# huggingface/open-muse

Measured on AMD Instinct MI355X. Metric: images/sec/node (MaskGit train step, 256^2, bs=64/GPU), higher is better.
Workload: dtype bf16 (transformer GEMM/attention operands; f32 accumulate, residual, norms, loss) + bf16x3 tokenizer (f32 activations, f32-class products as 3 bf16 MFMAs); parity of this mode was not measured in this run (a --full run measures it); 1 GPU; MaskGit train step: MaskGitVQGAN f16-256 encode (bf16x3) + cosine mask + MaskGitTransformer config B (configs/imagenet.yaml: hidden 768, 24 layers, 16 heads, vocab 2048, seq 257) fwd+bwd (bf16 MFMA, f32 accum/residual) + AdamW; global_batch=64, per_gpu_batch=64, resolution=256, seq_len=257, parallelism=dp1, vqgan_dtype=bf16x3, random_init=True, wgrad_stream=True

## Files before the change

### include/muse_hip.h

```cpp
#ifndef MUSE_HIP_H
#define MUSE_HIP_H
#include <stdint.h>

#ifdef __cplusplus
extern "C" {
#endif

enum { MUSE_F32 = 0, MUSE_BF16 = 1, MUSE_F16 = 2  };
enum { MUSE_ERR_BAD_ARG = -1, MUSE_ERR_ALIGN = -2, MUSE_ERR_UNSUPPORTED = -3 };

int muse_version(void);

typedef struct muse_gemm_desc {
  const void* A;
  const void* B;
  void* C;
  const void* bias;
  const void* rowvec;
  const void* residual;
  int32_t dtype;
  int32_t out_dtype;
  int32_t layout_a, layout_b;
  int32_t M, N, K;
  int32_t batch, zdiv;
// ... 32 lines not shown
int muse_colsum(const float* in, float* out, int32_t rows, int32_t cols, int32_t accumulate, void* stream);
int muse_add_rowvec(float* x, const float* b, int64_t rows, int32_t cols, void* stream);
int muse_bias_grad_rows_per_block(void);
int muse_bias_grad_partial(const void* dy, int32_t dtype, float* partial, int64_t rows, int32_t cols, int64_t ld, void* stream);

int muse_softmax_fwd(const void* x, void* y, int32_t dtype, int64_t rows, int32_t cols, int64_t ld, void* stream);
int muse_softmax_bwd(const void* p, const void* dp, void* ds, int32_t dtype, int64_t rows, int32_t cols, int64_t ld,
                     void* stream);

typedef struct muse_attn_desc {
  const void* q;
  const void* k;
  const void* v;
  void* o;
  int64_t ldq, ldk, ldv, ldo;
  int64_t bsq, bsk, bsv, bso;
  int32_t batch, heads, head_dim, seq_q, seq_kv;
  float alpha;
} muse_attn_desc;
int muse_attention_seq_pad(int32_t seq);
int muse_attention_fwd_ex(const muse_attn_desc* d, float* lse, void* stream);
int muse_attention_bwd_ex(const muse_attn_desc* d, const void* d_o, int64_t lddo, int64_t bsdo, const float* lse, float* dsum,
                          void* dq, int64_t lddq, int64_t bsdq, void* dk, int64_t lddk, int64_t bsdk, void* dv, int64_t lddv,
                          int64_t bsdv, void* stream);
int muse_attention_x3_fwd(const muse_attn_desc* d, float* lse, void* o_planes, int64_t o_lo, int32_t half, float scale, int32_t* stats,
                          void* stream);
int muse_attention_x3_bwd(const muse_attn_desc* d, const void* d_o, int64_t lddo, int64_t bsdo, const float* lse, void* dq,
                          int64_t lddq, int64_t bsdq, void* dk, int64_t lddk, int64_t bsdk, void* dv, int64_t lddv, int64_t bsdv,
                          void* dq_planes, int64_t dq_lo, void* dk_planes, int64_t dk_lo, void* dv_planes, int64_t dv_lo, int32_t half,
                          float scale, int32_t* stats, void* stream);
int muse_attention_x3_fwd_stream(const muse_attn_desc* d, float* lse, void* o_planes, int64_t o_lo, int32_t half, float scale,
                                 int32_t* stats, void* stream);
int muse_attention_x3_bwd_stream(const muse_attn_desc* d, const float* d_o, int64_t lddo, int64_t bsdo, const float* lse, float* dsum,
                                 float* dq, int64_t lddq, int64_t bsdq, float* dk, int64_t lddk, int64_t bsdk, float* dv, int64_t lddv,
                                 int64_t bsdv, void* dq_planes, int64_t dq_lo, void* dk_planes, int64_t dk_lo, void* dv_planes, int64_t dv_lo,
                                 int32_t half, float scale, int32_t* stats, void* stream);
int muse_attention_x3_merge(const float* part, int64_t part_stride, const float* lp, int64_t lp_stride, int32_t nk, float* out, float* lse,
                            void* out_planes, int64_t out_lo, int32_t batch, int32_t seq, int32_t heads, int32_t half, float scale,
                            int32_t* stats, void* stream);
int muse_sum_parts_strided(const float* parts, int64_t part_stride, int32_t n, int64_t rows, int32_t cols, float* out, int64_t ldo,
                           int32_t accumulate, void* stream);
int muse_attention_fwd(const void* qkv, void* ctx, float* lse, int32_t batch, int32_t seq, int32_t heads,
                       int32_t head_dim, float alpha, void* stream);
int muse_attention_bwd(const void* qkv, const void* ctx, const void* dctx, const float* lse, float* dsum, void* dqkv,
                       int32_t batch, int32_t seq, int32_t heads, int32_t head_dim, float alpha, void* stream);

int muse_glu_fwd(const void* ab, void* h, int32_t dtype, int64_t rows, int32_t inter, void* stream);
int muse_glu_bwd(const void* ab, const void* dh, void* dab, int32_t dtype, int64_t rows, int32_t inter, void* stream);
int muse_glu_fwd_x3(const float* ab, float* h, void* planes, int64_t rows, int32_t inter, int32_t half, float scale, int32_t* stats,
                    void* stream);
int muse_glu_bwd_x3(const float* ab, const float* dh, float* dab, void* planes, int64_t rows, int32_t inter, int32_t half, float scale,
                    int32_t* stats, void* stream);
int muse_ffn_mid_rows_per_block(void);
int muse_ffn_mid_fwd(const void* ab, const float* w, void* h, void* hm, float* mean, float* rstd, int32_t dtype,
                     int32_t rows, int32_t inter, float eps, void* stream);
int muse_ffn_mid_bwd(const void* dhm, const void* h, const void* ab, const float* w, const float* mean, const float* rstd,
                     void* dab, float* dw_partial, int32_t dtype, int32_t rows, int32_t inter, void* stream);
int muse_gelu_fwd(const void* x, void* y, int32_t dtype, int64_t n, void* stream);
int muse_gelu_bwd(const void* x, const void* dy, void* dx, int32_t dtype, int64_t n, void* stream);
int muse_gelu_bwd_f32_bf16(const float* x, const float* dy, void* dx_bf16, int64_t n, void* stream);

int muse_embed_fwd(const int64_t* ids, const float* word, const float* pos, float* out, int32_t batch, int32_t seq,
                   int32_t hidden, int32_t vocab, void* stream);
int muse_embed_bwd(const int64_t* ids, const float* dout, float* dword, float* dpos, float* scratch, int32_t batch,
                   int32_t seq, int32_t hidden, int32_t vocab, int32_t accumulate, void* stream);
int64_t muse_embed_bwd_scratch_floats(int32_t hidden, int32_t vocab);
int muse_embed_bwd2(const int64_t* ids, const float* dout, float* dword, float* dpos, void* scratch, int64_t scratch_bytes,
                    int32_t batch, int32_t seq, int32_t hidden, int32_t vocab, int32_t accumulate, void* stream);
int64_t muse_embed_bwd2_scratch_bytes(int32_t batch, int32_t seq, int32_t hidden, int32_t vocab);

int muse_cross_entropy_fwd(const void* logits, int32_t dtype, const int64_t* labels, float* row_loss, float* lse,
                           float* loss_out, int64_t rows, int32_t vocab, int64_t ld, float label_smoothing, void* stream);
int muse_cross_entropy_bwd(const void* logits, int32_t dtype, const int64_t* labels, const float* lse,
                           const float* loss_out, const float* grad_out, void* dlogits, int32_t dl_dtype, int64_t rows,
                           int32_t vocab, int64_t ld, float label_smoothing, void* stream);
int muse_soft_ce_fwd(const float* logits, const int64_t* labels, const float* soft, float* row_loss, float* lse, float* psum,
                     float* loss_out, int64_t rows, int32_t seq1, int32_t K, int64_t ld, void* stream);
int muse_soft_ce_bwd(const float* logits, const int64_t* labels, const float* soft, const float* lse, const float* psum,
                     const float* loss_out, const float* grad_out, void* dlogits, int32_t dl_dtype, int64_t rows, int32_t seq1,
                     int32_t K, int64_t ld, int64_t ldo, void* stream);

int muse_adamw_flat(float* p, const float* g, float* m, float* v, void* p_bf16, int64_t n, float lr, float beta1,
                    float beta2, float eps, float weight_decay, int32_t step, float grad_scale, const int32_t* skip, void* stream);
int muse_ema_multi(const int64_t* table, const int32_t* chunk_first, int32_t num_tensors, int32_t num_chunks, float one_minus_decay,
                   void* stream);
int muse_adamw_multi(const int64_t* table, const int32_t* chunk_first, int32_t num_tensors, int32_t num_chunks, float lr,
                     float beta1, float beta2, float eps, float weight_decay, int32_t step, float grad_scale, const int32_t* skip,
                     void* stream);
int muse_adamw_flat_groups(float* p, const float* g, float* m, float* v, void* p_bf16, int64_t n, int64_t base,
                           const int64_t* seg_end, const int32_t* seg_group, int32_t nseg, const float* group_hyper,
                           int32_t ngroups, int32_t step, float grad_scale, const int32_t* skip, void* stream);
int muse_adamw_multi_groups(const int64_t* table, const int32_t* chunk_first, int32_t num_tensors, int32_t num_chunks,
                            const float* group_hyper, int32_t ngroups, int32_t step, float grad_scale, const int32_t* skip, void* stream);

int muse_gradnorm_flat(const float* g_flat, int64_t base, int64_t n, const int64_t* ptab_host, const int32_t* chunk_first_host,
                       const int64_t* ptab, const int32_t* chunk_first, int32_t num_params, double* slab, void* stream);
int muse_gradnorm_multi(const int64_t* table, int32_t ncol, const int32_t* chunk_first, int32_t num_tensors, int32_t num_chunks,
                        double* slab, void* stream);
int muse_gradnorm_finalize(const double* slab, const int32_t* chunk_first, int32_t num_tensors, double* psum, float grad_scale,
                           float max_norm, float* out, void* stream);
int muse_grad_scale_flat(float* g, int64_t n, const float* scale, void* stream);
int muse_grad_scale_multi(const int64_t* table, int32_t ncol, const int32_t* chunk_first, int32_t num_tensors, int32_t num_chunks,
                          const float* scale, void* stream);
int muse_adamw_flat_dev(float* p, const float* g, float* m, float* v, void* p_bf16, int64_t n, float lr, float beta1, float beta2,
                        float eps, float weight_decay, int32_t step, const float* scale_dev, const int32_t* skip, void* stream);
int muse_adamw_multi_dev(const int64_t* table, const int32_t* chunk_first, int32_t num_tensors, int32_t num_chunks, float lr,
                         float beta1, float beta2, float eps, float weight_decay, int32_t step, const float* scale_dev,
                         const int32_t* skip, void* stream);
int muse_adamw_flat_groups_dev(float* p, const float* g, float* m, float* v, void* p_bf16, int64_t n, int64_t base,
                               const int64_t* seg_end, const int32_t* seg_group, int32_t nseg, const float* group_hyper,
                               int32_t ngroups, int32_t step, const float* scale_dev, const int32_t* skip, void* stream);
int muse_adamw_multi_groups_dev(const int64_t* table, const int32_t* chunk_first, int32_t num_tensors, int32_t num_chunks,
                                const float* group_hyper, int32_t ngroups, int32_t step, const float* scale_dev, const int32_t* skip,
                                void* stream);
int muse_sum_slices(const float* ws, float* out, int32_t nslices, int64_t n, int64_t stride, int32_t accumulate, void* stream);
int muse_sum_multi(const void* const* ws, void* const* out, const int32_t* nslices, const int64_t* n, const int64_t* stride,
                   const int32_t* accumulate, const int32_t* kind, int32_t njobs, void* stream);
int muse_split_f32_to_bf16x2(const float* in, void* hi, void* lo, int64_t n, void* stream);
int muse_sum_slices_epilogue(const float* ws, int32_t nslices, int64_t stride, const float* bias, const void* residual, int64_t ldr,
                             void* out, int32_t out_dtype, int64_t ldc, int64_t rows, int32_t cols, void* stream);
int muse_split_f32_to_bf16_cat3(const float* in, void* out, int64_t rows, int32_t cols, int64_t ld_in, int64_t ld_out, int32_t mode,
                                int32_t lo_pos, void* stream);
int muse_cast_f32_to_bf16(const float* in, void* out, int64_t n, void* stream);
int muse_cast_f32_to_f16(const float* in, void* out, int64_t n, float scale, int32_t* stats, void* stream);
int muse_cast_bf16_to_f32(const void* in, float* out, int64_t n, void* stream);

int muse_mask_sample(const int64_t* tokens, const int64_t* class_ids, const float* timesteps, const float* noise,
                     int64_t* input_ids, int64_t* labels, float* mask_prob, int32_t batch, int32_t seq, int64_t mask_id,
                     int64_t codebook_size, float min_masking_rate, void* stream);

int muse_sample_step(const float* cond_logits, const float* uncond_logits, float guidance_scale, int64_t img_stride, int64_t ld,
                     int32_t vocab,
                     const int64_t* input_ids, int64_t mask_id, const float* noise_exp, const float* noise_u, uint64_t seed,
                     uint32_t step, float temperature, int32_t sched_mask_len, int32_t batch, int32_t seq, int64_t* raw_sampled,
                     int64_t* sampled, int64_t* next_ids, float* conf_scratch, void* stream);

int muse_mask_tokens(const int64_t* tokens, const float* timesteps, const float* mask_prob_in, const float* noise,
                     const int32_t* rects, int64_t* input_ids, int64_t* labels, float* loss_weight, float* mask_prob,
                     int32_t batch, int32_t seq, int64_t mask_id, float min_masking_rate, int32_t all_labels, float weight_min,
                     void* stream);

int muse_dropout(const void* x, void* y, int32_t dtype, int64_t n, float p, uint64_t seed, uint64_t offset, void* stream);

int muse_cond_dropout(const float* x, const float* empty, const float* uniforms, float* out, int32_t batch, int64_t per_image,
                      float prob, void* stream);


int muse_conv2d_nhwc(const void* in, const void* weight, const float* bias, const void* residual, void* out,
                     int32_t dtype, int32_t batch, int32_t H, int32_t W, int32_t Cin, int32_t Cout, int32_t KS,
                     int32_t upsample, void* stream);
int muse_conv2d_nhwc_split(const float* in, const void* w_hi, const void* w_lo, const float* bias, const float* residual,
                           float* out, double* gn_partial, int32_t gn_groups, int32_t batch, int32_t H, int32_t W,
                           int32_t Cin, int32_t Cout, int32_t KS, int32_t upsample, void* stream);
int muse_conv2d_nhwc_split2(const void* in_hi, const void* in_lo, const void* w_hi, const void* w_lo, const float* bias,
                            const float* residual, float* out, double* gn_partial, int32_t gn_groups, int32_t batch,
                            int32_t H, int32_t W, int32_t Cin, int32_t Cout, int32_t KS, void* stream);
int muse_groupnorm_silu_nhwc(const void* x, void* y, int32_t dtype, const float* gamma, const float* beta,
                             double* partial, int32_t batch, int32_t HW, int32_t C, int32_t groups, float eps,
                             int32_t apply_silu, void* stream);
int muse_groupnorm_nchunk(int32_t HW);
int muse_conv2d_nhwc_gn_split2_ok(int32_t batch, int32_t H, int32_t W, int32_t Cin, int32_t Cout, int32_t KS);
int muse_conv2d_nhwc_gn_split2(const float* x, const float* gn_scale, const float* gn_shift, const void* w_hi, const void* w_lo,
                               const float* bias, const float* residual, float* out, double* gn_partial, int32_t gn_groups,
                               int32_t batch, int32_t H, int32_t W, int32_t Cin, int32_t Cout, int32_t KS, int32_t persistent,
                               void* stream);
int muse_conv2d_nhwc_gn_split2_pool(const float* x, const float* gn_scale, const float* gn_shift, const void* w_hi, const void* w_lo,
                                    const float* bias, const float* residual, float* out, double* gn_partial, int32_t gn_groups,
                                    int32_t batch, int32_t H, int32_t W, int32_t Cin, int32_t Cout, int32_t KS, int32_t persistent,
                                    void* stream);
int muse_groupnorm_scale_shift(const double* partial, int32_t nchunk, const float* gamma, const float* beta, float* scale,
                               float* shift, int32_t batch, int32_t HW, int32_t C, int32_t groups, float eps, void* stream);
int muse_conv_in_direct(const float* x, const float* w4, const float* bias, float* out, double* gn_partial, int32_t gn_groups,
                        int32_t batch, int32_t H, int32_t W, int32_t Cin, int32_t Cpad, int32_t Cout, void* stream);
int muse_conv_in_direct_nchw(const float* x, const float* w4, const float* bias, float* out, double* gn_partial, int32_t gn_groups,
                             int32_t batch, int32_t H, int32_t W, int32_t Cin, int32_t Cout, void* stream);
int muse_conv_out_direct(const float* x, const float* scale, const float* shift, const float* w, const float* bias, float* out,
                         int32_t batch, int32_t H, int32_t W, int32_t C, int32_t Cout, void* stream);
int muse_upsample2x_nhwc(const void* x, void* y, int32_t dtype, int32_t batch, int32_t H, int32_t W, int32_t C, void* stream);
int muse_upsample2x_split_nhwc(const float* x, void* y_hi, void* y_lo, int32_t batch, int32_t H, int32_t W, int32_t C, void* stream);
int muse_groupnorm_silu_nhwc_split(const float* x, void* y_hi, void* y_lo, const float* gamma, const float* beta,
                                   double* partial, int32_t stats_nchunk, int32_t batch, int32_t HW, int32_t C,
                                   int32_t groups, float eps, int32_t apply_silu, void* stream);
int muse_avgpool2x2_nhwc(const void* x, void* y, int32_t dtype, int32_t batch, int32_t H, int32_t W, int32_t C,
                         void* stream);
int muse_avgpool2x2_nhwc_stats(const float* x, float* y, double* partial, int32_t groups, int32_t batch, int32_t H, int32_t W,
                               int32_t C, void* stream);
int muse_nchw_to_nhwc(const float* in, void* out, int32_t out_dtype, int32_t batch, int32_t C, int32_t HW, int32_t Cpad,
                      void* stream);
int muse_nhwc_to_nchw(const void* in, int32_t in_dtype, float* out, int32_t batch, int32_t C, int32_t HW, int32_t Cpad,
                      void* stream);
int muse_argmin_rows(const float* dist, int64_t* idx, int64_t rows, int32_t ncodes, int64_t ld, void* stream);
int muse_row_sumsq(const float* x, float* out, int64_t rows, int32_t cols, int64_t ld, void* stream);
int muse_gather_rows(const float* table, const int64_t* idx, void* out, int32_t out_dtype, int64_t rows, int32_t cols,
                     void* stream);

int muse_probe_tr16(const int32_t* addr, int32_t* out, void* stream);

int muse_norm_res_fwd(const float* x, const float* res, const float* w, float* y, float* pre, int64_t rows, int32_t cols,
                      float eps, int32_t mode, void* stream);
int muse_adaln_fwd(const float* x, const float* ss, float* y, int32_t batch, int64_t rows_per_batch, int32_t C, void* stream);
int muse_adaln_fwd_ex(const float* x, const float* ss, float* y, void* y_bf16, int32_t batch, int64_t rows_per_batch, int32_t C,
                      void* stream);
int muse_silu_fwd(const float* x, float* y, int64_t n, void* stream);
int muse_dwconv3x3_nhwc(const float* x, const float* w, float* y, int32_t batch, int32_t H, int32_t W, int32_t C, void* stream);
int muse_space_to_depth2_nhwc(const float* x, float* y, int32_t batch, int32_t H, int32_t W, int32_t C, int32_t inverse, void* stream);
int muse_grn_fwd(const float* x, const float* gamma, const float* beta, float* y, float* scratch, int32_t batch, int64_t S,
                 int32_t C, void* stream);
int muse_grn_fwd_ex(const float* x, const float* gamma, const float* beta, float* y, void* y_bf16, float* scratch, int32_t batch,
                    int64_t S, int32_t C, void* stream);
int muse_sinusoidal_encode(const float* f, float* out, int64_t n, int32_t dim, float max_positions, void* stream);
int muse_weighted_mean(const float* v, const float* w, float* out, int64_t n, void* stream);
int muse_norm_res_bwd_nblk(int64_t rows);
int muse_norm_res_bwd(const float* dy, const float* dpre, const float* v, const float* w, float* dv, float* dw_partial,
                      int64_t rows, int32_t cols, float eps, int32_t mode, void* stream);
int muse_norm_res_bwd_ex(const float* dy, const float* dpre, const float* v, const float* w, float* dv, void* dv_bf16,
                         float* dw_partial, int64_t rows, int32_t cols, float eps, int32_t mode, void* stream);
int muse_norm_adaln_fwd(const float* x, const float* res, const float* w, const float* ss, float* pre, float* m, void* m_bf16,
                        int32_t batch, int64_t rows_per_batch, int32_t cols, float eps, int32_t mode, void* stream);
int muse_norm_adaln_bwd(const float* dm, const float* dpre, const float* v, const float* w, const float* ss, float* dv, void* dv_bf16,
                        float* dw_partial, float* dss_partial, int32_t batch, int64_t rows_per_batch, int32_t cols, float eps,
                        int32_t mode, void* stream);
int muse_norm_adaln_fwd_x3(const float* x, const float* res, const float* w, const float* ss, float* pre, float* m, void* planes,
                           int32_t batch, int64_t rows_per_batch, int32_t cols, float eps, int32_t mode, int32_t half, float scale,
                           int32_t* stats, void* stream);
int muse_norm_adaln_bwd_x3(const float* dm, const float* dpre, const float* v, const float* w, const float* ss, float* dv, void* planes,
                           float* dw_partial, float* dss_partial, int32_t batch, int64_t rows_per_batch, int32_t cols, float eps,
                           int32_t mode, int32_t half, float scale, int32_t* stats, void* stream);
int muse_colsum_segments(const float* part, float* out, int32_t nseg, int32_t seg_rows, int32_t cols, void* stream);
int muse_adaln_bwd(const float* dy, const float* x, const float* ss, float* dx, float* dss, int32_t batch,
                   int64_t rows_per_batch, int32_t C, void* stream);
int muse_silu_bwd(const float* x, const float* dy, float* dx, int64_t n, void* stream);
int muse_dwconv3x3_bwd_nchunk(int64_t pixels);
int muse_dwconv3x3_bwd(const float* dy, const float* x, const float* w, float* dx, float* dw_partial, int32_t batch, int32_t H,
                       int32_t W, int32_t C, void* stream);
int muse_grn_bwd(const float* dy, const float* x, const float* gamma, const float* stats, float* dx, float* work,
                 int32_t batch, int64_t S, int32_t C, void* stream);
int muse_scale_rows(float* x, const float* w, const float* num, const float* den, int64_t rows, int32_t cols, int64_t ld,
                    void* stream);

#ifdef __cplusplus
}
#endif
#endif
```

### open-muse_amd/csrc/conv_split.hip

```cpp
#include "gemm_core.h"
#include "../../include/muse_hip.h"

struct SplitParams {
  GemmParams g;
  const void* Blo;
  double* gn_partial;
  int gn_groups, gn_cpg;
};

__global__ __launch_bounds__(256, 2) void conv_split_kernel(SplitParams sp) {
  const GemmParams& p = sp.g;
  constexpr int BK = 64, IMG = 128 * 160;
  extern __shared__ __attribute__((aligned(16))) unsigned char smem[];
  unsigned char* tAh = smem;
  unsigned char* tAl = smem + IMG;
  unsigned char* tBh = smem + 2 * IMG;
  unsigned char* tBl = smem + 3 * IMG;

  const int ntm = (p.M + 127) >> 7, ntn = (p.N + 127) >> 7, ntiles = ntm * ntn;
  const int bq = ntiles >> 3, br = ntiles & 7, xcd = blockIdx.x & 7, bi = blockIdx.x >> 3;
  const int tid_ = (xcd < br ? xcd * (bq + 1) : br * (bq + 1) + (xcd - br) * bq) + bi;
  const int m0 = (tid_ / ntn) << 7, n0 = (tid_ % ntn) << 7;

  using ALoader = ConvLoader<float, 128, 256>;
// ... 15 lines not shown

  auto fetch = [&](int k0) {
#pragma unroll
    for (int i = 0; i < ALoader::NCH; ++i) ra[i] = la.load(i, k0);
#pragma unroll
    for (int i = 0; i < BLoader::NCH; ++i) { rh[i] = lh.load(i, k0); rl[i] = ll.load(i, k0); }
  };
  auto stage = [&]() {
#pragma unroll
    for (int i = 0; i < ALoader::NCH; ++i) {
      const int c = threadIdx.x + 256 * i;
      const int off = (c >> 4) * 160 + (c & 15) * 8;
      u32x2 hi, lo;
      split4(ra[i], hi, lo);
      *(u32x2*)(tAh + off) = hi;
      *(u32x2*)(tAl + off) = lo;
    }
#pragma unroll
    for (int i = 0; i < BLoader::NCH; ++i) {
      *(u32x4*)(tBh + BLoader::lds_off(i)) = rh[i];
      *(u32x4*)(tBl + BLoader::lds_off(i)) = rl[i];
    }
  };

  fetch(0);
  stage();
  __syncthreads();
  for (int kt = 0; kt < nk; ++kt) {
    const bool more = (kt + 1) < nk;
    if (more) fetch((kt + 1) * BK);
#pragma unroll
    for (int ks = 0; ks < 2; ++ks) {
      bf16x8 ah[4], al[4];
#pragma unroll
      for (int i = 0; i < 4; ++i) {
        ah[i] = frag_bf16<0, 128>(tAh, wr + i * 16, ks, lane);
        al[i] = frag_bf16<0, 128>(tAl, wr + i * 16, ks, lane);
      }
#pragma unroll
      for (int j = 0; j < 4; ++j) {
        const bf16x8 bh = frag_bf16<0, 128>(tBh, wc + j * 16, ks, lane);
        const bf16x8 bl = frag_bf16<0, 128>(tBl, wc + j * 16, ks, lane);
#pragma unroll
        for (int i = 0; i < 4; ++i) {
          acc[i][j] = __builtin_amdgcn_mfma_f32_16x16x32_bf16(bl, ah[i], acc[i][j], 0, 0, 0);
          acc[i][j] = __builtin_amdgcn_mfma_f32_16x16x32_bf16(bh, al[i], acc[i][j], 0, 0, 0);
          acc[i][j] = __builtin_amdgcn_mfma_f32_16x16x32_bf16(bh, ah[i], acc[i][j], 0, 0, 0);
        }
      }
    }
    __syncthreads();
    if (more) {
      stage();
      __syncthreads();
    }
  }

  float* Cp = (float*)p.C;
  const float* Rp = (const float*)p.residual;
  const bool vec_ok = ((p.ldc & 3) == 0) && ((((uintptr_t)Cp) & 15) == 0) &&
                      (Rp == nullptr || (((p.ldr & 3) == 0) && ((((uintptr_t)Rp) & 15) == 0)));
  double gs[4] = {0.0, 0.0, 0.0, 0.0}, gq[4] = {0.0, 0.0, 0.0, 0.0};
#pragma unroll
  for (int i = 0; i < 4; ++i) {
    const int m = m0 + wr + i * 16 + (lane & 15);
    if (m >= p.M) continue;
#pragma unroll
    for (int j = 0; j < 4; ++j) {
      const int n = n0 + wc + j * 16 + 4 * (lane >> 4);
      if (n >= p.N) continue;
      float v[4];
#pragma unroll
      for (int r = 0; r < 4; ++r) v[r] = acc[i][j][r] + ((p.bias && (n + r) < p.N) ? p.bias[n + r] : 0.f);
      float* cptr = Cp + (long)m * p.ldc + n;
      if (vec_ok && (n + 3) < p.N) {
        if (Rp) { float t[4]; OutVec<float>::load4(Rp + (long)m * p.ldr + n, t); v[0] += t[0]; v[1] += t[1]; v[2] += t[2]; v[3] += t[3]; }
        OutVec<float>::store4(cptr, v);
        if (sp.gn_partial) {
#pragma unroll
          for (int r = 0; r < 4; ++r) { gs[j] += (double)v[r]; gq[j] += (double)v[r] * (double)v[r]; }
        }
      } else {
#pragma unroll
        for (int r = 0; r < 4; ++r)
          if ((n + r) < p.N) cptr[r] = v[r] + (Rp ? Rp[(long)m * p.ldr + n + r] : 0.f);
      }
    }
  }
  if (sp.gn_partial) {
#pragma unroll
    for (int j = 0; j < 4; ++j)
#pragma unroll
      for (int o = 1; o < 16; o <<= 1) { gs[j] += __shfl_xor(gs[j], o, 64); gq[j] += __shfl_xor(gq[j], o, 64); }
    double* red = (double*)smem;
    if ((lane & 15) == 0) {
#pragma unroll
      for (int j = 0; j < 4; ++j) {
        const int chunk = (wc >> 2) + j * 4 + (lane >> 4);
        red[((wave >> 1) * 32 + chunk) * 2] = gs[j];
        red[((wave >> 1) * 32 + chunk) * 2 + 1] = gq[j];
      }
    }
    __syncthreads();
    if (threadIdx.x < 32) {
      double cs = red[threadIdx.x * 2] + red[(32 + threadIdx.x) * 2];
      double cq = red[threadIdx.x * 2 + 1] + red[(32 + threadIdx.x) * 2 + 1];
      const int cpc = sp.gn_cpg >> 2;
      for (int o = 1; o < cpc; o <<= 1) { cs += __shfl_xor(cs, o, 64); cq += __shfl_xor(cq, o, 64); }
      const int n = n0 + (int)threadIdx.x * 4;
      if ((threadIdx.x & (cpc - 1)) == 0 && n < p.N) {
        const int hw = p.cH * p.cW, b = m0 / hw, chunk = (m0 - b * hw) >> 7, nchunk = hw >> 7;
        double* o2 = sp.gn_partial + (((long)b * nchunk + chunk) * sp.gn_groups + n / sp.gn_cpg) * 2;
        o2[0] = cs; o2[1] = cq;
      }
    }
  }
}

extern "C" int muse_conv2d_nhwc_split(const float* in, const void* w_hi, const void* w_lo, const float* bias,
                                      const float* residual, float* out, double* gn_partial, int32_t gn_groups, int32_t batch,
                                      int32_t H, int32_t W, int32_t Cin, int32_t Cout, int32_t KS, int32_t upsample,
                                      void* stream) {
  if (Cin % 8) return MUSE_ERR_ALIGN;
  if ((((uintptr_t)in) & 15) || (((uintptr_t)w_hi) & 15) || (((uintptr_t)w_lo) & 15)) return MUSE_ERR_ALIGN;
  if (KS != 1 && KS != 3) return MUSE_ERR_UNSUPPORTED;
  if (upsample < 0 || upsample > 2 || (upsample == 2 && KS != 3)) return MUSE_ERR_BAD_ARG;
  if (upsample == 1 && ((H | W) & 1)) return MUSE_ERR_BAD_ARG;
  SplitParams sp;
  sp.gn_partial = nullptr; sp.gn_groups = 0; sp.gn_cpg = 0;
  if (gn_partial) {
    const int cpg = gn_groups > 0 ? Cout / gn_groups : 0;
    if (gn_groups <= 0 || (Cout % gn_groups) || (cpg & 3) || cpg > 32 || (cpg & (cpg - 1)) || ((H * W) & 127) || (Cout & 3) ||
        (((uintptr_t)out) & 15) || (((uintptr_t)residual) & 15))
      return MUSE_ERR_UNSUPPORTED;
    sp.gn_partial = gn_partial; sp.gn_groups = gn_groups; sp.gn_cpg = cpg;
  }
  GemmParams& p = sp.g;
  p.A = in; p.B = w_hi; p.C = out; sp.Blo = w_lo;
  p.bias = bias; p.rowvec = nullptr; p.residual = residual;
  p.M = batch * H * W; p.N = Cout; p.K = KS * KS * Cin;
  p.lda = 0; p.ldb = p.K; p.ldc = Cout; p.ldr = Cout;
  p.zdiv = 1; p.sA0 = p.sA1 = p.sB0 = p.sB1 = p.sC0 = p.sC1 = 0;
  p.alpha = 1.0f; p.accumulate = 0; p.act = 0; p.split_k = 1; p.split_stride = 0;
  p.cH = H; p.cW = W; p.cCin = Cin; p.cKS = KS; p.cUps = upsample;
  p.cCinShift = -1;
  if ((Cin & (Cin - 1)) == 0) { int sh = 0; while ((1 << sh) < Cin) ++sh; p.cCinShift = sh; }
  if (p.M <= 0 || p.N <= 0) return 0;
  const int ntm = (p.M + 127) / 128, ntn = (p.N + 127) / 128;
  const size_t lds = 4 * 128 * 160;
  set_max_dynamic_lds((const void*)conv_split_kernel, lds);
  hipLaunchKernelGGL(conv_split_kernel, dim3(ntm * ntn), dim3(256), lds, (hipStream_t)stream, sp);
  return (int)hipGetLastError();
}
```

### open-muse_amd/csrc/gemm_core.h

```cpp
#pragma once
#include "common.h"
#include <stdlib.h>

struct GemmParams {
  const void* A;
  const void* B;
  void* C;
  const float* bias;
  const float* rowvec;
  const void* residual;
  int M, N, K;
  long lda, ldb, ldc, ldr;
  int zdiv;
  long sA0, sA1, sB0, sB1, sC0, sC1;
  float alpha;
  int accumulate;
  int act;
  int split_k;
  long split_stride;
  int cH, cW, cCin, cKS, cUps, cCinShift;
  long a_lo, b_lo;
};

template <typename T> struct TileCfg;
// ... 45 lines not shown
    for (int i = 0; i < NCH; ++i) {
      const int c = threadIdx.x + NT * i;
      if (LAYOUT == 0) {
        const int row = r0 + c / CPR, col = (c % CPR) * Cfg::CH;
        voff[i] = row < R ? (unsigned)(((long)row * ld + col) * E) : oob;
      } else {
        const int kr = c / CPR, r = r0 + (c % CPR) * Cfg::CH;
        voff[i] = r < R ? (unsigned)(((long)kr * ld + r) * E) : oob;
      }
    }
  }
  __device__ __forceinline__ u32x4 load(int i, int k0) const {
    const int c = threadIdx.x + NT * i;
    const int kk = k0 + (LAYOUT == 0 ? (c % CPR) * Cfg::CH : c / CPR);
    return buf_load16(rs, kk < K ? voff[i] : oob, (unsigned)k0 * kstep);
  }
  static __device__ __forceinline__ int lds_off(int i) {
    const int c = threadIdx.x + NT * i;
    if (LAYOUT == 0) {
      return (c / CPR) * Cfg::KC_STRIDE + (c % CPR) * 16;
    } else {
      int kr = c / CPR;
      if (sizeof(T) == 2) kr = km_phys_row_bf16(kr);
      return kr * KmCfg<T, ROWS>::STRIDE + (c % CPR) * 16;
    }
  }
};

template <typename T, int ROWS, int NT>
struct ConvLoader {
  using Cfg = TileCfg<T>;
  static constexpr int CPR = Cfg::BK / Cfg::CH;
  static constexpr int NCH = ROWS * Cfg::BK * (int)sizeof(T) / 16 / NT;
  rsrc_t rs;
  unsigned center[NCH], tapmask[NCH], pyx[NCH];
  unsigned oob;
  int iw, Cin, KS, ups, cshift, padv;
  __device__ __forceinline__ void init(const void* ptr, long, int R_, int K_, int r0_, const GemmParams& p) {
    constexpr int E = (int)sizeof(T);
    const int H = p.cH, W = p.cW;
    Cin = p.cCin; KS = p.cKS; ups = p.cUps; cshift = p.cCinShift;
    const int ih = ups == 1 ? (H >> 1) : ups == 2 ? (H << 1) : H;
    iw = ups == 1 ? (W >> 1) : ups == 2 ? (W << 1) : W;
    const unsigned bytes = (unsigned)((long)(R_ / (H * W)) * ih * iw * Cin * E);
    rs = make_rsrc(ptr, bytes);
    oob = (bytes + 15u) & ~15u;
    const int pad = (KS - 1) >> 1;
    padv = ups == 2 ? 0 : pad;
#pragma unroll
    for (int i = 0; i < NCH; ++i) {
      const int c = threadIdx.x + NT * i;
      const int m = r0_ + c / CPR;
      const int b = m / (H * W), rem = m - b * (H * W);
      const int y = rem / W, x = rem - y * W;
      unsigned mask = 0;
      if (m < R_) {
        for (int t = 0; t < KS * KS; ++t) {
          const int ky = t / KS, kx = t - ky * KS;
          if (ups == 2) {
            if (2 * y + ky < ih && 2 * x + kx < iw) mask |= 1u << t;
          } else {
            const int iy = y + ky - pad, ix = x + kx - pad;
            if (iy >= 0 && iy < H && ix >= 0 && ix < W) mask |= 1u << t;
          }
        }
      }
      tapmask[i] = mask;
      pyx[i] = (unsigned)y | ((unsigned)x << 16);
      center[i] = ups == 1 ? (unsigned)(b * ih * iw)
                : ups == 2 ? (unsigned)(((long)(b * ih + 2 * y) * iw + 2 * x) * Cin * E)
                           : (unsigned)(((long)(b * H + y) * W + x) * Cin * E);
    }
  }
  __device__ __forceinline__ u32x4 load(int i, int k0) const {
    constexpr int E = (int)sizeof(T);
    const int c = threadIdx.x + NT * i;
    const int k = k0 + (c % CPR) * Cfg::CH;
    const int kpos = cshift >= 0 ? (k >> cshift) : (k / Cin), ci = k - kpos * Cin;
    const int ky = KS == 3 ? ((kpos * 11) >> 5) : 0, kx = kpos - ky * KS;
    const bool ok = kpos < 9 && ((tapmask[i] >> kpos) & 1u);
    unsigned off;
    if (ups != 1) {
      off = center[i] + (unsigned)((((ky - padv) * iw + (kx - padv)) * Cin + ci) * E);
    } else {
      const int pad = (KS - 1) >> 1;
      const int iy = ((int)(pyx[i] & 0xffffu) + ky - pad) >> 1, ix = ((int)(pyx[i] >> 16) + kx - pad) >> 1;
      off = (unsigned)(((long)(center[i] + (unsigned)(iy * iw + ix)) * Cin + ci) * E);
    }
    return buf_load16(rs, ok ? off : oob, 0u);
  }
  static __device__ __forceinline__ int lds_off(int i) {
    const int c = threadIdx.x + NT * i;
    return (c / CPR) * Cfg::KC_STRIDE + (c % CPR) * 16;
  }
};

template <int LAYOUT, int ROWS>
__device__ __forceinline__ bf16x8 frag_bf16(const unsigned char* tile, int rowbase, int ks, int lane) {
  if (LAYOUT == 0) {
    return *(const bf16x8*)(tile + (rowbase + (lane & 15)) * TileCfg<bf16_t>::KC_STRIDE + ks * 64 + (lane >> 4) * 16);
  } else {
    const int p = lane & 15, g = lane >> 4;
    const int kr = ks * 32 + 8 * g + (p >> 2);
    const int col = (rowbase + (p & 3) * 4) * 2;
    typedef __attribute__((address_space(3))) s16x4 lds_s16x4;
    const unsigned char* a0 = tile + km_phys_row_bf16(kr) * KmCfg<bf16_t, ROWS>::STRIDE + col;
    const unsigned char* a1 = tile + km_phys_row_bf16(kr + 4) * KmCfg<bf16_t, ROWS>::STRIDE + col;
    union { s16x4 h[2]; bf16x8 v; } u;
    u.h[0] = __builtin_amdgcn_ds_read_tr16_b64_v4i16((lds_s16x4*)a0);
    u.h[1] = __builtin_amdgcn_ds_read_tr16_b64_v4i16((lds_s16x4*)a1);
    return u.v;
  }
}

template <int LAYOUT, int ROWS>
__device__ __forceinline__ f32x4 frag_f32(const unsigned char* tile, int rowbase, int ks, int lane) {
  if (LAYOUT == 0) {
    return *(const f32x4*)(tile + (rowbase + (lane & 15)) * TileCfg<float>::KC_STRIDE + ks * 64 + (lane >> 4) * 16);
  } else {
    constexpr int ST = KmCfg<float, ROWS>::STRIDE;
    const unsigned char* q = tile + (16 * ks + 4 * (lane >> 4)) * ST + (rowbase + (lane & 15)) * 4;
    f32x4 v;
    v[0] = *(const float*)(q);
    v[1] = *(const float*)(q + ST);
    v[2] = *(const float*)(q + 2 * ST);
    v[3] = *(const float*)(q + 3 * ST);
    return v;
  }
}

template <typename TC> struct OutVec;
template <> struct OutVec<float> {
  static __device__ __forceinline__ void load4(const float* p, float (&v)[4]) {
    const f32x4 t = *(const f32x4*)p; v[0] = t[0]; v[1] = t[1]; v[2] = t[2]; v[3] = t[3];
  }
  static __device__ __forceinline__ void store4(float* p, const float (&v)[4]) {
    f32x4 t = {v[0], v[1], v[2], v[3]}; *(f32x4*)p = t;
  }
};
template <> struct OutVec<bf16_t> {
  static __device__ __forceinline__ void load4(const bf16_t* p, float (&v)[4]) {
    const u32x2 t = *(const u32x2*)p;
    v[0] = __uint_as_float(t[0] << 16); v[1] = __uint_as_float(t[0] & 0xffff0000u);
    v[2] = __uint_as_float(t[1] << 16); v[3] = __uint_as_float(t[1] & 0xffff0000u);
  }
  static __device__ __forceinline__ void store4(bf16_t* p, const float (&v)[4]) {
    u32x2 t;
    t[0] = pack2_bf16(v[0], v[1]);
    t[1] = pack2_bf16(v[2], v[3]);
    *(u32x2*)p = t;
  }
};

template <typename T, typename TC, int AL, int BL, int BM, int NSTAGE, typename ALoader, typename BLoader>
__global__ __launch_bounds__(BM * 2, 2) void gemm_kernel(GemmParams p) {
  using Cfg = TileCfg<T>;
  constexpr int TA_BYTES = TileBytes<T, BM>::VALUE, TB_BYTES = TileBytes<T, 128>::VALUE;
  extern __shared__ __attribute__((aligned(16))) unsigned char smem[];
  unsigned char* tA = smem;
  unsigned char* tB = smem + TA_BYTES;
  constexpr int STAGE_BYTES = TA_BYTES + TB_BYTES;

  const int ntm = (p.M + BM - 1) / BM, ntn = (p.N + 127) >> 7, ntiles = ntm * ntn;
  const int bq = ntiles >> 3, br = ntiles & 7, xcd = blockIdx.x & 7, bi = blockIdx.x >> 3;
  const int tid_ = (xcd < br ? xcd * (bq + 1) : br * (bq + 1) + (xcd - br) * bq) + bi;
  constexpr int GM = 1024 / BM;
  const int grp = tid_ / (GM * ntn), first_m = grp * GM;
  const int gm = min(ntm - first_m, GM), in_grp = tid_ - grp * (GM * ntn);
  const int m0 = (first_m + in_grp % gm) * BM, n0 = (in_grp / gm) << 7;

  const int z = blockIdx.z, zq = z / p.zdiv, zr = z - zq * p.zdiv;
  const T* Ap = (const T*)p.A + zq * p.sA0 + zr * p.sA1;
  const T* Bp = (const T*)p.B + zq * p.sB0 + zr * p.sB1;
  TC* Cp = (TC*)p.C + zq * p.sC0 + zr * p.sC1 + (p.split_k > 1 ? (long)blockIdx.y * p.split_stride : 0L);
  const bool atomic_out = p.split_k > 1 && p.split_stride == 0;

  int nk = (p.K + Cfg::BK - 1) / Cfg::BK, kt0 = 0;
  if (p.split_k > 1) {
    const int per = (nk + p.split_k - 1) / p.split_k;
    kt0 = blockIdx.y * per;
    nk = min(nk, kt0 + per);
    if (kt0 >= nk) return;
  }
  const int kend = min(p.K, nk * Cfg::BK);
  ALoader la; la.init(Ap, p.lda, p.M, kend, m0, p);
  BLoader lb; lb.init(Bp, p.ldb, p.N, kend, n0, p);

  const int lane = threadIdx.x & 63, wave = threadIdx.x >> 6;
  const int wr = (wave >> 1) * 64, wc = (wave & 1) * 64;

  f32x4 acc[4][4];
#pragma unroll
  for (int i = 0; i < 4; ++i)
#pragma unroll
    for (int j = 0; j < 4; ++j) acc[i][j] = f32x4{0.f, 0.f, 0.f, 0.f};

  auto compute = [&](const unsigned char* cA, const unsigned char* cB) {
    if constexpr (sizeof(T) == 2) {
#pragma unroll
      for (int ks = 0; ks < 2; ++ks) {
        bf16x8 af[4], bf[4];
#pragma unroll
        for (int i = 0; i < 4; ++i) {
          af[i] = frag_bf16<AL, BM>(cA, wr + i * 16, ks, lane);
          bf[i] = frag_bf16<BL, 128>(cB, wc + i * 16, ks, lane);
        }
#pragma unroll
        for (int i = 0; i < 4; ++i)
#pragma unroll
          for (int j = 0; j < 4; ++j)
            acc[i][j] = __builtin_amdgcn_mfma_f32_16x16x32_bf16(bf[j], af[i], acc[i][j], 0, 0, 0);
      }
    } else {
#pragma unroll
      for (int ks = 0; ks < Cfg::BK / 16; ++ks) {
        f32x4 af[4], bf[4];
#pragma unroll
        for (int i = 0; i < 4; ++i) {
          af[i] = frag_f32<AL, BM>(cA, wr + i * 16, ks, lane);
          bf[i] = frag_f32<BL, 128>(cB, wc + i * 16, ks, lane);
        }
#pragma unroll
        for (int s = 0; s < 4; ++s)
#pragma unroll
          for (int i = 0; i < 4; ++i)
#pragma unroll
            for (int j = 0; j < 4; ++j)
              acc[i][j] = __builtin_amdgcn_mfma_f32_16x16x4f32(bf[j][s], af[i][s], acc[i][j], 0, 0, 0);
      }
    }
  };

  if constexpr (NSTAGE == 1) {
    u32x4 ra[ALoader::NCH], rb[BLoader::NCH];
#pragma unroll
    for (int i = 0; i < ALoader::NCH; ++i) ra[i] = la.load(i, kt0 * Cfg::BK);
#pragma unroll
    for (int i = 0; i < BLoader::NCH; ++i) rb[i] = lb.load(i, kt0 * Cfg::BK);
#pragma unroll
    for (int i = 0; i < ALoader::NCH; ++i) *(u32x4*)(tA + ALoader::lds_off(i)) = ra[i];
#pragma unroll
    for (int i = 0; i < BLoader::NCH; ++i) *(u32x4*)(tB + BLoader::lds_off(i)) = rb[i];
    __syncthreads();
    for (int kt = kt0; kt < nk; ++kt) {
      const bool more = (kt + 1) < nk;
      if (more) {
#pragma unroll
        for (int i = 0; i < ALoader::NCH; ++i) ra[i] = la.load(i, (kt + 1) * Cfg::BK);
#pragma unroll
        for (int i = 0; i < BLoader::NCH; ++i) rb[i] = lb.load(i, (kt + 1) * Cfg::BK);
      }
      compute(tA, tB);
      __syncthreads();
      if (more) {
#pragma unroll
        for (int i = 0; i < ALoader::NCH; ++i) *(u32x4*)(tA + ALoader::lds_off(i)) = ra[i];
#pragma unroll
        for (int i = 0; i < BLoader::NCH; ++i) *(u32x4*)(tB + BLoader::lds_off(i)) = rb[i];
        __syncthreads();
      }
    }
  } else {
    u32x4 ra0[ALoader::NCH], rb0[BLoader::NCH], ra1[ALoader::NCH], rb1[BLoader::NCH];
    unsigned char* tA1 = tA + STAGE_BYTES;
    unsigned char* tB1 = tB + STAGE_BYTES;
#define MUSE_FETCH(RA, RB, KT)                                                          \
  {                                                                                     \
    _Pragma("unroll") for (int i = 0; i < ALoader::NCH; ++i) RA[i] = la.load(i, (KT) * Cfg::BK); \
    _Pragma("unroll") for (int i = 0; i < BLoader::NCH; ++i) RB[i] = lb.load(i, (KT) * Cfg::BK); \
  }
#define MUSE_STAGE(RA, RB, DA, DB)                                                      \
  {                                                                                     \
    _Pragma("unroll") for (int i = 0; i < ALoader::NCH; ++i) *(u32x4*)((DA) + ALoader::lds_off(i)) = RA[i]; \
    _Pragma("unroll") for (int i = 0; i < BLoader::NCH; ++i) *(u32x4*)((DB) + BLoader::lds_off(i)) = RB[i]; \
  }
    const int nk2 = kt0 + ((nk - kt0 + 1) & ~1);
    MUSE_FETCH(ra0, rb0, kt0)
    MUSE_FETCH(ra1, rb1, kt0 + 1)
    MUSE_STAGE(ra0, rb0, tA, tB)
    __syncthreads();
    for (int kt = kt0; kt < nk2; kt += 2) {
      MUSE_FETCH(ra0, rb0, kt + 2)
      __builtin_amdgcn_sched_barrier(0);
      compute(tA, tB);
      MUSE_STAGE(ra1, rb1, tA1, tB1)
      __syncthreads();
      MUSE_FETCH(ra1, rb1, kt + 3)
      __builtin_amdgcn_sched_barrier(0);
      compute(tA1, tB1);
      MUSE_STAGE(ra0, rb0, tA, tB)
      __syncthreads();
    }
#undef MUSE_FETCH
#undef MUSE_STAGE
  }

  if constexpr (BM == 128) {
    constexpr int EPC = 16 / (int)sizeof(TC);
    constexpr int CST = 128 * (int)sizeof(TC) + 16;
    const bool fast = !atomic_out && (p.N % EPC) == 0 && (p.ldc % EPC) == 0 && ((((uintptr_t)Cp) & 15) == 0) &&
                      (p.residual == nullptr || (((p.ldr % EPC) == 0) && ((((uintptr_t)p.residual) & 15) == 0)));
    if (fast) {
      constexpr int NH = sizeof(TC) == 4 ? 2 : 1, RPP = 128 / NH;
      constexpr int CPRo = 128 / EPC;
      const TC* Rq = (const TC*)p.residual;
#pragma unroll
      for (int half = 0; half < NH; ++half) {
        __syncthreads();
        if (wr / RPP == half) {
#pragma unroll
          for (int i = 0; i < 4; ++i) {
            const int ml = wr + i * 16 + (lane & 15);
            const float rv = (p.rowvec && (m0 + ml) < p.M) ? p.rowvec[m0 + ml] : 0.f;
#pragma unroll
            for (int j = 0; j < 4; ++j) {
              const int nl = wc + j * 16 + 4 * (lane >> 4);
              float v[4];
#pragma unroll
              for (int r = 0; r < 4; ++r) {
                float add = rv;
                if (p.bias && (n0 + nl + r) < p.N) add += p.bias[n0 + nl + r];
                float x = p.alpha * acc[i][j][r] + add;
                if (p.act == 1) x = gelu_erf(x);
                v[r] = x;
              }
              OutVec<TC>::store4((TC*)(smem + (ml - half * RPP) * CST) + nl, v);
            }
          }
        }
        __syncthreads();
#pragma unroll
        for (int it = 0; it < (RPP * CPRo) / 256; ++it) {
          const int c = threadIdx.x + 256 * it;
          const int row = c / CPRo, col = (c % CPRo) * EPC;
          const int m = m0 + half * RPP + row, n = n0 + col;
          if (m < p.M && n < p.N) {
            u32x4 w = *(const u32x4*)(smem + row * CST + col * (int)sizeof(TC));
            if (Rq || p.accumulate) {
              float o[EPC];
              if constexpr (sizeof(TC) == 4) {
#pragma unroll
                for (int e = 0; e < 4; ++e) o[e] = __uint_as_float(w[e]);
              } else {
#pragma unroll
                for (int e = 0; e < 4; ++e) { o[2 * e] = __uint_as_float(w[e] << 16); o[2 * e + 1] = __uint_as_float(w[e] & 0xffff0000u); }
              }
              auto add16 = [&](const TC* src) {
                const u32x4 t = *(const u32x4*)src;
                if constexpr (sizeof(TC) == 4) {
#pragma unroll
                  for (int e = 0; e < 4; ++e) o[e] += __uint_as_float(t[e]);
                } else {
#pragma unroll
                  for (int e = 0; e < 4; ++e) { o[2 * e] += __uint_as_float(t[e] << 16); o[2 * e + 1] += __uint_as_float(t[e] & 0xffff0000u); }
                }
              };
              if (Rq) add16(Rq + (long)m * p.ldr + n);
              if (p.accumulate) add16(Cp + (long)m * p.ldc + n);
              if constexpr (sizeof(TC) == 4) {
#pragma unroll
                for (int e = 0; e < 4; ++e) w[e] = __float_as_uint(o[e]);
              } else {
#pragma unroll
                for (int e = 0; e < 4; ++e) w[e] = pack2_bf16(o[2 * e], o[2 * e + 1]);
              }
            }
            *(u32x4*)(Cp + (long)m * p.ldc + n) = w;
          }
        }
      }
      return;
    }
  }
  const bool vec_ok = ((p.ldc & 3) == 0) && ((((uintptr_t)Cp) & 15) == 0) &&
                      (p.residual == nullptr || (((p.ldr & 3) == 0) && ((((uintptr_t)p.residual) & 15) == 0)));
  const TC* Rp = (const TC*)p.residual;
#pragma unroll
  for (int i = 0; i < 4; ++i) {
    const int m = m0 + wr + i * 16 + (lane & 15);
    if (m >= p.M) continue;
    const float rv = p.rowvec ? p.rowvec[m] : 0.f;
#pragma unroll
    for (int j = 0; j < 4; ++j) {
      const int n = n0 + wc + j * 16 + 4 * (lane >> 4);
      if (n >= p.N) continue;
      float v[4];
#pragma unroll
      for (int r = 0; r < 4; ++r) {
        float add = rv;
        if (p.bias && (n + r) < p.N) add += p.bias[n + r];
        float x = p.alpha * acc[i][j][r] + add;
        if (p.act == 1) x = gelu_erf(x);
        v[r] = x;
      }
      TC* cptr = Cp + (long)m * p.ldc + n;
      if constexpr (sizeof(TC) == 4) {
        if (atomic_out) {
#pragma unroll
          for (int r = 0; r < 4; ++r)
            if ((n + r) < p.N) unsafeAtomicAdd((float*)cptr + r, v[r]);
          continue;
        }
      }
      if (vec_ok && (n + 3) < p.N) {
        if (Rp) { float t[4]; OutVec<TC>::load4(Rp + (long)m * p.ldr + n, t); v[0] += t[0]; v[1] += t[1]; v[2] += t[2]; v[3] += t[3]; }
        if (p.accumulate) { float t[4]; OutVec<TC>::load4(cptr, t); v[0] += t[0]; v[1] += t[1]; v[2] += t[2]; v[3] += t[3]; }
        OutVec<TC>::store4(cptr, v);
      } else {
#pragma unroll
        for (int r = 0; r < 4; ++r) {
          if ((n + r) < p.N) {
            float x = v[r];
            if (Rp) x += Elem<TC>::load(Rp + (long)m * p.ldr + n + r);
            if (p.accumulate) x += Elem<TC>::load(cptr + r);
            Elem<TC>::store(cptr + r, x);
          }
        }
      }
    }
  }
}

template <typename T, typename TC, int AL, int BL, int BM, int NSTAGE, typename ALoader, typename BLoader>
static inline int launch_gemm_st(const GemmParams& p, int batch, hipStream_t stream) {
  const int ntm = (p.M + BM - 1) / BM, ntn = (p.N + 127) / 128;
  dim3 grid(ntm * ntn, p.split_k > 1 ? p.split_k : 1, batch);
  constexpr size_t tiles = (size_t)NSTAGE * (TileBytes<T, BM>::VALUE + TileBytes<T, 128>::VALUE);
  constexpr size_t ctile = BM == 128 ? (size_t)(sizeof(TC) == 4 ? 64 : 128) * (128 * sizeof(TC) + 16) : 0;
  constexpr size_t lds = tiles > ctile ? tiles : ctile;
  auto kern = gemm_kernel<T, TC, AL, BL, BM, NSTAGE, ALoader, BLoader>;
  set_max_dynamic_lds((const void*)kern, lds);
  hipLaunchKernelGGL(kern, grid, dim3(BM * 2), lds, stream, p);
  return (int)hipGetLastError();
}

static inline int gemm_stages(int al, int bl) {
  static const int st = [] { const char* e = getenv("MUSE_GEMM_STAGES"); return e ? (e[0] == '1' ? 1 : 2) : 0; }();
  if (st) return st;
  return (al == 0 && bl == 0) ? 1 : 2;
}
template <typename T, typename TC, int AL, int BL, int BM, typename ALoader, typename BLoader>
static inline int launch_gemm(const GemmParams& p, int batch, hipStream_t stream) {
  if (p.M <= 0 || p.N <= 0 || batch <= 0) return 0;
  if constexpr (sizeof(T) == 2) {
    if (gemm_stages(AL, BL) == 2) return launch_gemm_st<T, TC, AL, BL, BM, 2, ALoader, BLoader>(p, batch, stream);
  }
  return launch_gemm_st<T, TC, AL, BL, BM, 1, ALoader, BLoader>(p, batch, stream);
}

static inline bool use_bm256(const GemmParams& p, int batch) {
  static const int enabled = [] { const char* e = getenv("MUSE_BM256"); return (e && e[0] == '1') ? 1 : 0; }();
  if (!enabled) return false;
  const long tiles256 = (long)((p.M + 255) / 256) * ((p.N + 127) / 128) * batch * (p.split_k > 1 ? p.split_k : 1);
  return p.M >= 1024 && tiles256 >= 512;
}
```

### open-muse_amd/csrc/vqgan.hip

```cpp
#include "gemm_core.h"
#include "../../include/muse_hip.h"

extern "C" int muse_conv2d_nhwc(const void* in, const void* weight, const float* bias, const void* residual, void* out,
                                int32_t dtype, int32_t batch, int32_t H, int32_t W, int32_t Cin, int32_t Cout, int32_t KS,
                                int32_t upsample, void* stream) {
  const int esz = dtype == MUSE_BF16 ? 2 : 4, ch = 16 / esz;
  if (Cin % ch) return MUSE_ERR_ALIGN;
  if ((((uintptr_t)in) & 15) || (((uintptr_t)weight) & 15)) return MUSE_ERR_ALIGN;
  if (KS != 1 && KS != 3) return MUSE_ERR_UNSUPPORTED;
  if (upsample < 0 || upsample > 2 || (upsample == 2 && KS != 3)) return MUSE_ERR_BAD_ARG;
  if (upsample == 1 && ((H | W) & 1)) return MUSE_ERR_BAD_ARG;
  GemmParams p;
  p.A = in; p.B = weight; p.C = out;
  p.bias = bias; p.rowvec = nullptr; p.residual = residual;
  p.M = batch * H * W; p.N = Cout; p.K = KS * KS * Cin;
  p.lda = 0; p.ldb = p.K; p.ldc = Cout; p.ldr = Cout;
  p.zdiv = 1; p.sA0 = p.sA1 = p.sB0 = p.sB1 = p.sC0 = p.sC1 = 0;
  p.alpha = 1.0f; p.accumulate = 0; p.act = 0; p.split_k = 1; p.split_stride = 0;
  p.cH = H; p.cW = W; p.cCin = Cin; p.cKS = KS; p.cUps = upsample;
  p.cCinShift = -1;
  if ((Cin & (Cin - 1)) == 0) { int sh = 0; while ((1 << sh) < Cin) ++sh; p.cCinShift = sh; }
  hipStream_t s = (hipStream_t)stream;
  const bool big = use_bm256(p, 1);
  if (dtype == MUSE_BF16)
// ... 573 lines not shown
                                          void* stream) {
  if (C & 7) return MUSE_ERR_UNSUPPORTED;
  if ((((uintptr_t)x) | ((uintptr_t)y_hi) | ((uintptr_t)y_lo)) & 15) return MUSE_ERR_ALIGN;
  const long npix = (long)batch * H * W;
  if (npix <= 0) return 0;
  long g = (npix * (C >> 3) + 255) / 256; if (g > 65536) g = 65536;
  hipLaunchKernelGGL(upsample2x_split_kernel, dim3((unsigned)g), dim3(256), 0, (hipStream_t)stream, x, (bf16_t*)y_hi, (bf16_t*)y_lo, npix, H, W, C);
  return (int)hipGetLastError();
}

template <typename T, int VEC>
__global__ void avgpool_kernel(const T* __restrict__ x, T* __restrict__ y, int B, int H, int W, int C) {
  const int oh = H >> 1, ow = W >> 1, vpp = C / VEC;
  const long n = (long)B * oh * ow * vpp;
  for (long i = (long)blockIdx.x * blockDim.x + threadIdx.x; i < n; i += (long)gridDim.x * blockDim.x) {
    const int vc = (int)(i % vpp);
    long t = i / vpp;
    const int ox = (int)(t % ow); t /= ow;
    const int oy = (int)(t % oh);
    const int b = (int)(t / oh);
    const T* src = x + (((long)b * H + 2 * oy) * W + 2 * ox) * C + vc * VEC;
    float a[VEC], c0[VEC], c1[VEC], c2[VEC];
    loadv<T, VEC>(src, a); loadv<T, VEC>(src + C, c0); loadv<T, VEC>(src + (long)W * C, c1); loadv<T, VEC>(src + (long)W * C + C, c2);
#pragma unroll
    for (int j = 0; j < VEC; ++j) a[j] = (((a[j] + c0[j]) + c1[j]) + c2[j]) * 0.25f;
    storev<T, VEC>(y + (((long)b * oh + oy) * ow + ox) * C + vc * VEC, a);
  }
}
extern "C" int muse_avgpool2x2_nhwc(const void* x, void* y, int32_t dtype, int32_t batch, int32_t H, int32_t W, int32_t C,
                                    void* stream) {
  const int vec = dtype == MUSE_BF16 ? 8 : 4;
  if ((C % vec) || ((H | W) & 1)) return MUSE_ERR_BAD_ARG;
  const long n = (long)batch * (H / 2) * (W / 2) * (C / vec);
  if (n <= 0) return 0;
  long g = (n + 255) / 256; if (g > 8192) g = 8192;
  if (dtype == MUSE_F32) hipLaunchKernelGGL((avgpool_kernel<float, 4>), dim3((int)g), dim3(256), 0, (hipStream_t)stream, (const float*)x, (float*)y, batch, H, W, C);
  else hipLaunchKernelGGL((avgpool_kernel<bf16_t, 8>), dim3((int)g), dim3(256), 0, (hipStream_t)stream, (const bf16_t*)x, (bf16_t*)y, batch, H, W, C);
  return (int)hipGetLastError();
}

__global__ __launch_bounds__(256) void avgpool_stats_kernel(const float* __restrict__ x, float* __restrict__ y,
                                                            double* __restrict__ partial, int H, int W, int C, int G) {
  __shared__ double gs[64], gq[64];
  const int chunk = blockIdx.x, b = blockIdx.y, nchunk = gridDim.x;
  if (threadIdx.x < G) { gs[threadIdx.x] = 0.0; gq[threadIdx.x] = 0.0; }
  __syncthreads();
  const int oh = H >> 1, ow = W >> 1, oHW = oh * ow, vpp = C >> 2, cpg = C / G;
  const int p0 = chunk * GN_PIX_PER_CHUNK, p1 = min(oHW, p0 + GN_PIX_PER_CHUNK);
  const int vc = threadIdx.x % vpp, ppi = 256 / vpp;
  double s[4] = {0.0, 0.0, 0.0, 0.0}, q[4] = {0.0, 0.0, 0.0, 0.0};
  constexpr int UN = 2;
  for (int pb = p0 + threadIdx.x / vpp; pb < p1; pb += UN * ppi) {
    float a[UN][4], c0[UN][4], c1[UN][4], c2[UN][4];
#pragma unroll
    for (int u = 0; u < UN; ++u) {
      const int p = pb + u * ppi;
      if (p < p1) {
        const int oy = p / ow, ox = p - oy * ow;
        const float* src = x + (((long)b * H + 2 * oy) * W + 2 * ox) * C + vc * 4;
        loadv<float, 4>(src, a[u]); loadv<float, 4>(src + C, c0[u]);
        loadv<float, 4>(src + (long)W * C, c1[u]); loadv<float, 4>(src + (long)W * C + C, c2[u]);
      }
    }
#pragma unroll
    for (int u = 0; u < UN; ++u) {
      const int p = pb + u * ppi;
      if (p >= p1) break;
#pragma unroll
      for (int j = 0; j < 4; ++j) {
        a[u][j] = (((a[u][j] + c0[u][j]) + c1[u][j]) + c2[u][j]) * 0.25f;
        s[j] += (double)a[u][j]; q[j] += (double)a[u][j] * (double)a[u][j];
      }
      storev<float, 4>(y + ((long)b * oHW + p) * C + vc * 4, a[u]);
    }
  }
#pragma unroll
  for (int j = 0; j < 4; ++j) {
    const int g = (vc * 4 + j) / cpg;
    atomicAdd(&gs[g], s[j]); atomicAdd(&gq[g], q[j]);
  }
  __syncthreads();
  if (threadIdx.x < G) {
    double* o = partial + (((long)b * nchunk + chunk) * G + threadIdx.x) * 2;
    o[0] = gs[threadIdx.x]; o[1] = gq[threadIdx.x];
  }
}
extern "C" int muse_avgpool2x2_nhwc_stats(const float* x, float* y, double* partial, int32_t groups, int32_t batch, int32_t H,
                                          int32_t W, int32_t C, void* stream) {
  if ((C % 4) || ((H | W) & 1)) return MUSE_ERR_BAD_ARG;
  const int vpp = C / 4;
  if ((groups != 32 && groups != 64) || (C % groups) || vpp > 256 || (256 % vpp)) return MUSE_ERR_UNSUPPORTED;
  if (batch <= 0 || H <= 0 || W <= 0) return 0;
  const int nchunk = muse_groupnorm_nchunk((H / 2) * (W / 2));
  hipLaunchKernelGGL(avgpool_stats_kernel, dim3(nchunk, batch), dim3(256), 0, (hipStream_t)stream, x, y, partial, H, W, C, groups);
  return (int)hipGetLastError();
}

template <typename T>
__global__ void nchw_to_nhwc_kernel(const float* __restrict__ in, T* __restrict__ out, int C, int HW, int Cpad, long npix) {
  for (long i = (long)blockIdx.x * blockDim.x + threadIdx.x; i < npix; i += (long)gridDim.x * blockDim.x) {
    const long b = i / HW; const int p = (int)(i - b * HW);
    for (int c = 0; c < Cpad; ++c) {
      const float v = c < C ? in[(b * C + c) * HW + p] : 0.f;
      Elem<T>::store(out + i * Cpad + c, v);
    }
  }
}
template <typename T>
__global__ void nhwc_to_nchw_kernel(const T* __restrict__ in, float* __restrict__ out, int C, int HW, int Cpad, long npix) {
  for (long i = (long)blockIdx.x * blockDim.x + threadIdx.x; i < npix; i += (long)gridDim.x * blockDim.x) {
    const long b = i / HW; const int p = (int)(i - b * HW);
    for (int c = 0; c < C; ++c) out[(b * C + c) * HW + p] = Elem<T>::load(in + i * Cpad + c);
  }
}
extern "C" int muse_nchw_to_nhwc(const float* in, void* out, int32_t out_dtype, int32_t batch, int32_t C, int32_t HW,
                                 int32_t Cpad, void* stream) {
  const long npix = (long)batch * HW;
  if (npix <= 0) return 0;
  long g = (npix + 255) / 256; if (g > 8192) g = 8192;
  if (out_dtype == MUSE_F32) hipLaunchKernelGGL(nchw_to_nhwc_kernel<float>, dim3((int)g), dim3(256), 0, (hipStream_t)stream, in, (float*)out, C, HW, Cpad, npix);
  else hipLaunchKernelGGL(nchw_to_nhwc_kernel<bf16_t>, dim3((int)g), dim3(256), 0, (hipStream_t)stream, in, (bf16_t*)out, C, HW, Cpad, npix);
  return (int)hipGetLastError();
}
extern "C" int muse_nhwc_to_nchw(const void* in, int32_t in_dtype, float* out, int32_t batch, int32_t C, int32_t HW,
                                 int32_t Cpad, void* stream) {
  const long npix = (long)batch * HW;
  if (npix <= 0) return 0;
  long g = (npix + 255) / 256; if (g > 8192) g = 8192;
  if (in_dtype == MUSE_F32) hipLaunchKernelGGL(nhwc_to_nchw_kernel<float>, dim3((int)g), dim3(256), 0, (hipStream_t)stream, (const float*)in, out, C, HW, Cpad, npix);
  else hipLaunchKernelGGL(nhwc_to_nchw_kernel<bf16_t>, dim3((int)g), dim3(256), 0, (hipStream_t)stream, (const bf16_t*)in, out, C, HW, Cpad, npix);
  return (int)hipGetLastError();
}

__global__ __launch_bounds__(256) void argmin_rows_kernel(const float* __restrict__ d, int64_t* __restrict__ idx, long rows, int n, long ld) {
  const int lane = threadIdx.x & 63;
  const long row = (long)blockIdx.x * 4 + (threadIdx.x >> 6);
  if (row >= rows) return;
  const float* r = d + row * ld;
  float best = INFINITY; int bi = 0x7fffffff;
  for (int c = lane; c < n; c += 64) { const float v = r[c]; if (v < best) { best = v; bi = c; } }
#pragma unroll
  for (int o = 32; o > 0; o >>= 1) {
    const float ov = __shfl_xor(best, o, 64); const int oi = __shfl_xor(bi, o, 64);
    if (ov < best || (ov == best && oi < bi)) { best = ov; bi = oi; }
  }
  if (lane == 0) idx[row] = (int64_t)bi;
}
extern "C" int muse_argmin_rows(const float* dist, int64_t* idx, int64_t rows, int32_t ncodes, int64_t ld, void* stream) {
  if (rows <= 0) return 0;
  hipLaunchKernelGGL(argmin_rows_kernel, dim3((unsigned)((rows + 3) / 4)), dim3(256), 0, (hipStream_t)stream, dist, idx, (long)rows, ncodes, (long)ld);
  return (int)hipGetLastError();
}

__global__ __launch_bounds__(256) void row_sumsq_kernel(const float* __restrict__ x, float* __restrict__ out, long rows, int cols, long ld) {
  const int lane = threadIdx.x & 63;
  const long row = (long)blockIdx.x * 4 + (threadIdx.x >> 6);
  if (row >= rows) return;
  double s = 0.0;
  for (int c = lane; c < cols; c += 64) { const double v = (double)x[row * ld + c]; s += v * v; }
  s = wave_sum_d(s);
  if (lane == 0) out[row] = (float)s;
}
extern "C" int muse_row_sumsq(const float* x, float* out, int64_t rows, int32_t cols, int64_t ld, void* stream) {
  if (rows <= 0) return 0;
  hipLaunchKernelGGL(row_sumsq_kernel, dim3((unsigned)((rows + 3) / 4)), dim3(256), 0, (hipStream_t)stream, x, out, (long)rows, cols, (long)ld);
  return (int)hipGetLastError();
}

template <typename T>
__global__ void gather_rows_kernel(const float* __restrict__ table, const int64_t* __restrict__ idx, T* __restrict__ out, long rows, int cols) {
  const long r = blockIdx.x;
  const int64_t id = idx[r];
  for (int c = threadIdx.x; c < cols; c += blockDim.x) Elem<T>::store(out + r * cols + c, table[id * cols + c]);
}
extern "C" int muse_gather_rows(const float* table, const int64_t* idx, void* out, int32_t out_dtype, int64_t rows, int32_t cols,
                                void* stream) {
  if (rows <= 0) return 0;
  if (out_dtype == MUSE_F32) hipLaunchKernelGGL(gather_rows_kernel<float>, dim3((unsigned)rows), dim3(64), 0, (hipStream_t)stream, table, idx, (float*)out, (long)rows, cols);
  else hipLaunchKernelGGL(gather_rows_kernel<bf16_t>, dim3((unsigned)rows), dim3(64), 0, (hipStream_t)stream, table, idx, (bf16_t*)out, (long)rows, cols);
  return (int)hipGetLastError();
}

template <typename T>
__global__ __launch_bounds__(256) void transpose_kernel(const T* __restrict__ in, T* __restrict__ out, int rows, int cols, long ldi,
                                                        long ldo, long si, long so) {
  __shared__ T tile[32][33];
  const T* ib = in + (long)blockIdx.z * si;
  T* ob = out + (long)blockIdx.z * so;
  const int c0 = blockIdx.x * 32, r0 = blockIdx.y * 32;
  const int tx = threadIdx.x & 31, ty = threadIdx.x >> 5;
  for (int j = ty; j < 32; j += 8) {
    const int r = r0 + j, c = c0 + tx;
    if (r < rows && c < cols) tile[j][tx] = ib[(long)r * ldi + c];
  }
  __syncthreads();
  for (int j = ty; j < 32; j += 8) {
    const int c = c0 + j, r = r0 + tx;
    if (r < rows && c < cols) ob[(long)c * ldo + r] = tile[tx][j];
  }
}
extern "C" int muse_transpose(const void* in, void* out, int32_t dtype, int32_t rows, int32_t cols, int64_t ld_in,
                              int64_t ld_out, int32_t batch, int64_t stride_in, int64_t stride_out, void* stream) {
  if (rows <= 0 || cols <= 0 || batch <= 0) return 0;
  dim3 grid((cols + 31) / 32, (rows + 31) / 32, batch);
  if (dtype == MUSE_F32) hipLaunchKernelGGL(transpose_kernel<float>, grid, dim3(256), 0, (hipStream_t)stream, (const float*)in, (float*)out, rows, cols, (long)ld_in, (long)ld_out, (long)stride_in, (long)stride_out);
  else hipLaunchKernelGGL(transpose_kernel<bf16_t>, grid, dim3(256), 0, (hipStream_t)stream, (const bf16_t*)in, (bf16_t*)out, rows, cols, (long)ld_in, (long)ld_out, (long)stride_in, (long)stride_out);
  return (int)hipGetLastError();
}

__global__ void probe_tr16_kernel(const int* __restrict__ addr, int* __restrict__ out) {
  __shared__ __attribute__((aligned(16))) unsigned short lds[8192];
  for (int i = threadIdx.x; i < 8192; i += 64) lds[i] = (unsigned short)i;
  __syncthreads();
  typedef __attribute__((address_space(3))) s16x4 lds_s16x4;
  const unsigned char* a = (const unsigned char*)lds + addr[threadIdx.x];
  const s16x4 r = __builtin_amdgcn_ds_read_tr16_b64_v4i16((lds_s16x4*)a);
#pragma unroll
  for (int j = 0; j < 4; ++j) out[threadIdx.x * 4 + j] = (int)(unsigned short)r[j];
}
extern "C" int muse_probe_tr16(const int32_t* addr, int32_t* out, void* stream) {
  hipLaunchKernelGGL(probe_tr16_kernel, dim3(1), dim3(64), 0, (hipStream_t)stream, addr, out);
  return (int)hipGetLastError();
}
```

### open-muse_amd/muse/_hip.py

```python
from __future__ import annotations

import ctypes as C
import os

import torch

F32, BF16, F16 = 0, 1, 2
_HERE = os.path.dirname(os.path.abspath(__file__))
LIB_PATH = os.environ.get("MUSE_HIP_LIB") or os.path.join(_HERE, "libmuse_hip.so")
_lib = None

c_void_p, c_int, c_i64, c_float = C.c_void_p, C.c_int32, C.c_int64, C.c_float


class GemmDesc(C.Structure):
    _fields_ = [
        ("A", c_void_p), ("B", c_void_p), ("C", c_void_p),
        ("bias", c_void_p), ("rowvec", c_void_p), ("residual", c_void_p),
        ("dtype", c_int), ("out_dtype", c_int), ("layout_a", c_int), ("layout_b", c_int),
        ("M", c_int), ("N", c_int), ("K", c_int), ("batch", c_int), ("zdiv", c_int),
        ("lda", c_i64), ("ldb", c_i64), ("ldc", c_i64), ("ldr", c_i64),
        ("sA0", c_i64), ("sA1", c_i64), ("sB0", c_i64), ("sB1", c_i64), ("sC0", c_i64), ("sC1", c_i64),
        ("alpha", c_float), ("accumulate", c_int), ("act", c_int), ("split_k", c_int), ("split_stride", c_i64),
    ]


class AttnDesc(C.Structure):
    _fields_ = [
        ("q", c_void_p), ("k", c_void_p), ("v", c_void_p), ("o", c_void_p),
        ("ldq", c_i64), ("ldk", c_i64), ("ldv", c_i64), ("ldo", c_i64),
        ("bsq", c_i64), ("bsk", c_i64), ("bsv", c_i64), ("bso", c_i64),
        ("batch", c_int), ("heads", c_int), ("head_dim", c_int), ("seq_q", c_int), ("seq_kv", c_int),
        ("alpha", c_float),
    ]


_IMG = (c_int, c_float, c_void_p)

SIGNATURES = {
    "muse_version": [],
    "muse_gemm": [C.POINTER(GemmDesc), c_void_p],
    "muse_gemm_x3": [C.POINTER(GemmDesc), c_i64, c_i64, c_void_p],
    "muse_gemm_tile": [C.POINTER(GemmDesc)],
    "muse_gemm_path": [C.POINTER(GemmDesc)],
    "muse_transpose": [c_void_p, c_void_p, c_int, c_int, c_int, c_i64, c_i64, c_int, c_i64, c_i64, c_void_p],
    "muse_layernorm_fwd": [c_void_p, c_int, c_void_p, c_void_p, c_void_p, c_int, c_void_p, c_void_p, c_int, c_int,
                           c_float, c_void_p],
    "muse_layernorm_bwd": [c_void_p, c_int, c_void_p, c_int, c_void_p, c_void_p, c_void_p, c_void_p, c_void_p, c_int,
                           c_void_p, c_void_p, c_int, c_int, c_int, c_void_p],
    "muse_layernorm_bwd_nblk": [c_int],
    "muse_layernorm_pair_fwd": [c_void_p] * 10 + [c_int, c_int, c_float, c_void_p],
    "muse_layernorm_pair_bwd": [c_void_p] * 14 + [c_int, c_int, c_int, c_void_p],
    "muse_colsum": [c_void_p, c_void_p, c_int, c_int, c_int, c_void_p],
    "muse_add_rowvec": [c_void_p, c_void_p, c_i64, c_int, c_void_p],
    "muse_bias_grad_rows_per_block": [],
    "muse_bias_grad_partial": [c_void_p, c_int, c_void_p, c_i64, c_int, c_i64, c_void_p],
    "muse_softmax_fwd": [c_void_p, c_void_p, c_int, c_i64, c_int, c_i64, c_void_p],
    "muse_softmax_bwd": [c_void_p, c_void_p, c_void_p, c_int, c_i64, c_int, c_i64, c_void_p],
    "muse_attention_seq_pad": [c_int],
    "muse_attention_fwd_ex": [C.POINTER(AttnDesc), c_void_p, c_void_p],
    "muse_attention_bwd_ex": [C.POINTER(AttnDesc), c_void_p, c_i64, c_i64, c_void_p, c_void_p, c_void_p, c_i64, c_i64, c_void_p,
                              c_i64, c_i64, c_void_p, c_i64, c_i64, c_void_p],
    "muse_attention_x3_fwd": [C.POINTER(AttnDesc), c_void_p, c_void_p, c_i64, *_IMG, c_void_p],
    "muse_attention_x3_bwd": [C.POINTER(AttnDesc), c_void_p, c_i64, c_i64, c_void_p, c_void_p, c_i64, c_i64, c_void_p, c_i64, c_i64, c_void_p,
                              c_i64, c_i64, c_void_p, c_i64, c_void_p, c_i64, c_void_p, c_i64, *_IMG, c_void_p],
    "muse_attention_x3_fwd_stream": [C.POINTER(AttnDesc), c_void_p, c_void_p, c_i64, *_IMG, c_void_p],
    "muse_attention_x3_bwd_stream": [C.POINTER(AttnDesc), c_void_p, c_i64, c_i64, c_void_p, c_void_p, c_void_p, c_i64, c_i64, c_void_p, c_i64, c_i64,
                                     c_void_p, c_i64, c_i64, c_void_p, c_i64, c_void_p, c_i64, c_void_p, c_i64, *_IMG, c_void_p],
    "muse_attention_x3_merge": [c_void_p, c_i64, c_void_p, c_i64, c_int, c_void_p, c_void_p, c_void_p, c_i64, c_int, c_int, c_int, *_IMG,
                                c_void_p],
    "muse_sum_parts_strided": [c_void_p, c_i64, c_int, c_i64, c_int, c_void_p, c_i64, c_int, c_void_p],
    "muse_attention_fwd": [c_void_p, c_void_p, c_void_p, c_int, c_int, c_int, c_int, c_float, c_void_p],
    "muse_attention_bwd": [c_void_p, c_void_p, c_void_p, c_void_p, c_void_p, c_void_p, c_int, c_int, c_int, c_int, c_float,
                           c_void_p],
    "muse_glu_fwd": [c_void_p, c_void_p, c_int, c_i64, c_int, c_void_p],
    "muse_glu_bwd": [c_void_p, c_void_p, c_void_p, c_int, c_i64, c_int, c_void_p],
    "muse_glu_fwd_x3": [c_void_p, c_void_p, c_void_p, c_i64, c_int, *_IMG, c_void_p],
    "muse_glu_bwd_x3": [c_void_p, c_void_p, c_void_p, c_void_p, c_i64, c_int, *_IMG, c_void_p],
    "muse_ffn_mid_rows_per_block": [],
    "muse_ffn_mid_fwd": [c_void_p, c_void_p, c_void_p, c_void_p, c_void_p, c_void_p, c_int, c_int, c_int, c_float, c_void_p],
    "muse_ffn_mid_bwd": [c_void_p, c_void_p, c_void_p, c_void_p, c_void_p, c_void_p, c_void_p, c_void_p, c_int, c_int, c_int,
                         c_void_p],
    "muse_gelu_fwd": [c_void_p, c_void_p, c_int, c_i64, c_void_p],
    "muse_gelu_bwd": [c_void_p, c_void_p, c_void_p, c_int, c_i64, c_void_p],
    "muse_gelu_bwd_f32_bf16": [c_void_p, c_void_p, c_void_p, c_i64, c_void_p],
    "muse_embed_fwd": [c_void_p, c_void_p, c_void_p, c_void_p, c_int, c_int, c_int, c_int, c_void_p],
    "muse_embed_bwd": [c_void_p, c_void_p, c_void_p, c_void_p, c_void_p, c_int, c_int, c_int, c_int, c_int, c_void_p],
    "muse_embed_bwd_scratch_floats": [c_int, c_int],
    "muse_embed_bwd2": [c_void_p, c_void_p, c_void_p, c_void_p, c_void_p, c_i64, c_int, c_int, c_int, c_int, c_int, c_void_p],
    "muse_embed_bwd2_scratch_bytes": [c_int, c_int, c_int, c_int],
    "muse_cross_entropy_fwd": [c_void_p, c_int, c_void_p, c_void_p, c_void_p, c_void_p, c_i64, c_int, c_i64, c_float,
                               c_void_p],
    "muse_cross_entropy_bwd": [c_void_p, c_int, c_void_p, c_void_p, c_void_p, c_void_p, c_void_p, c_int, c_i64, c_int,
                               c_i64, c_float, c_void_p],
    "muse_soft_ce_fwd": [c_void_p, c_void_p, c_void_p, c_void_p, c_void_p, c_void_p, c_void_p, c_i64, c_int, c_int, c_i64, c_void_p],
    "muse_soft_ce_bwd": [c_void_p, c_void_p, c_void_p, c_void_p, c_void_p, c_void_p, c_void_p, c_void_p, c_int, c_i64, c_int, c_int,
                         c_i64, c_i64, c_void_p],
    "muse_adamw_flat": [c_void_p, c_void_p, c_void_p, c_void_p, c_void_p, c_i64, c_float, c_float, c_float, c_float,
                        c_float, c_int, c_float, c_void_p, c_void_p],
    "muse_adamw_multi": [c_void_p, c_void_p, c_int, c_int, c_float, c_float, c_float, c_float, c_float, c_int, c_float, c_void_p,
                         c_void_p],
    "muse_ema_multi": [c_void_p, c_void_p, c_int, c_int, c_float, c_void_p],
    "muse_adamw_flat_groups": [c_void_p, c_void_p, c_void_p, c_void_p, c_void_p, c_i64, c_i64, c_void_p, c_void_p, c_int, c_void_p,
                               c_int, c_int, c_float, c_void_p, c_void_p],
    "muse_adamw_multi_groups": [c_void_p, c_void_p, c_int, c_int, c_void_p, c_int, c_int, c_float, c_void_p, c_void_p],
    "muse_gradnorm_flat": [c_void_p, c_i64, c_i64, c_void_p, c_void_p, c_void_p, c_void_p, c_int, c_void_p, c_void_p],
    "muse_gradnorm_multi": [c_void_p, c_int, c_void_p, c_int, c_int, c_void_p, c_void_p],
    "muse_gradnorm_finalize": [c_void_p, c_void_p, c_int, c_void_p, c_float, c_float, c_void_p, c_void_p],
    "muse_grad_scale_flat": [c_void_p, c_i64, c_void_p, c_void_p],
    "muse_grad_scale_multi": [c_void_p, c_int, c_void_p, c_int, c_int, c_void_p, c_void_p],
    "muse_adamw_flat_dev": [c_void_p, c_void_p, c_void_p, c_void_p, c_void_p, c_i64, c_float, c_float, c_float, c_float,
                            c_float, c_int, c_void_p, c_void_p, c_void_p],
    "muse_adamw_multi_dev": [c_void_p, c_void_p, c_int, c_int, c_float, c_float, c_float, c_float, c_float, c_int, c_void_p, c_void_p,
                             c_void_p],
    "muse_adamw_flat_groups_dev": [c_void_p, c_void_p, c_void_p, c_void_p, c_void_p, c_i64, c_i64, c_void_p, c_void_p, c_int, c_void_p,
                                   c_int, c_int, c_void_p, c_void_p, c_void_p],
    "muse_adamw_multi_groups_dev": [c_void_p, c_void_p, c_int, c_int, c_void_p, c_int, c_int, c_void_p, c_void_p, c_void_p],
    "muse_gemm_group_ok": [c_void_p, c_int, c_int],
    "muse_gemm_group": [c_void_p, c_int, c_int, c_void_p],
    "muse_sum_multi": [c_void_p, c_void_p, c_void_p, c_void_p, c_void_p, c_void_p, c_void_p, c_int, c_void_p],
    "muse_conv_out_direct": [c_void_p, c_void_p, c_void_p, c_void_p, c_void_p, c_void_p, c_int, c_int, c_int, c_int, c_int, c_void_p],
    "muse_upsample2x_split_nhwc": [c_void_p, c_void_p, c_void_p, c_int, c_int, c_int, c_int, c_void_p],
    "muse_split_f32_to_bf16x2": [c_void_p, c_void_p, c_void_p, c_i64, c_void_p],
    "muse_upsample2x_nhwc": [c_void_p, c_void_p, c_int, c_int, c_int, c_int, c_int, c_void_p],
    "muse_sum_slices_epilogue": [c_void_p, c_int, c_i64, c_void_p, c_void_p, c_i64, c_void_p, c_int, c_i64, c_i64, c_int, c_void_p],
    "muse_split_f32_to_bf16_cat3": [c_void_p, c_void_p, c_i64, c_int, c_i64, c_i64, c_int, c_int, c_void_p],
    "muse_sum_slices": [c_void_p, c_void_p, c_int, c_i64, c_i64, c_int, c_void_p],
    "muse_cast_f32_to_bf16": [c_void_p, c_void_p, c_i64, c_void_p],
    "muse_cast_bf16_to_f32": [c_void_p, c_void_p, c_i64, c_void_p],
    "muse_cast_f32_to_f16": [c_void_p, c_void_p, c_i64, c_float, c_void_p, c_void_p],
    "muse_mask_sample": [c_void_p, c_void_p, c_void_p, c_void_p, c_void_p, c_void_p, c_void_p, c_int, c_int, c_i64,
                         c_i64, c_float, c_void_p],
    "muse_sample_step": [c_void_p, c_void_p, c_float, c_i64, c_i64, c_int, c_void_p, c_i64, c_void_p, c_void_p, C.c_uint64, C.c_uint32,
                         c_float, c_int, c_int, c_int, c_void_p, c_void_p, c_void_p, c_void_p, c_void_p],
    "muse_mask_tokens": [c_void_p, c_void_p, c_void_p, c_void_p, c_void_p, c_void_p, c_void_p, c_void_p, c_void_p, c_int, c_int,
                         c_i64, c_float, c_int, c_float, c_void_p],
    "muse_dropout": [c_void_p, c_void_p, c_int, c_i64, c_float, C.c_uint64, C.c_uint64, c_void_p],
    "muse_cond_dropout": [c_void_p, c_void_p, c_void_p, c_void_p, c_int, c_i64, c_float, c_void_p],
    "muse_conv2d_nhwc": [c_void_p, c_void_p, c_void_p, c_void_p, c_void_p, c_int, c_int, c_int, c_int, c_int, c_int,
                         c_int, c_int, c_void_p],
    "muse_conv2d_nhwc_split": [c_void_p, c_void_p, c_void_p, c_void_p, c_void_p, c_void_p, c_void_p, c_int, c_int, c_int, c_int,
                               c_int, c_int, c_int, c_int, c_void_p],
    "muse_conv2d_nhwc_split2": [c_void_p, c_void_p, c_void_p, c_void_p, c_void_p, c_void_p, c_void_p, c_void_p, c_int, c_int, c_int,
                                c_int, c_int, c_int, c_int, c_void_p],
    "muse_conv_in_direct": [c_void_p, c_void_p, c_void_p, c_void_p, c_void_p, c_int, c_int, c_int, c_int, c_int, c_int, c_int, c_void_p],
    "muse_conv_in_direct_nchw": [c_void_p, c_void_p, c_void_p, c_void_p, c_void_p, c_int, c_int, c_int, c_int, c_int, c_int, c_void_p],
    "muse_conv2d_nhwc_gn_split2_ok": [c_int, c_int, c_int, c_int, c_int, c_int],
    "muse_conv2d_nhwc_gn_split2": [c_void_p] * 9 + [c_int] * 8 + [c_void_p],
    "muse_conv2d_nhwc_gn_split2_pool": [c_void_p] * 9 + [c_int] * 8 + [c_void_p],
    "muse_groupnorm_scale_shift": [c_void_p, c_int, c_void_p, c_void_p, c_void_p, c_void_p, c_int, c_int, c_int, c_int, c_float, c_void_p],
    "muse_groupnorm_silu_nhwc_split": [c_void_p, c_void_p, c_void_p, c_void_p, c_void_p, c_void_p, c_int, c_int, c_int, c_int,
                                       c_int, c_float, c_int, c_void_p],
    "muse_groupnorm_silu_nhwc": [c_void_p, c_void_p, c_int, c_void_p, c_void_p, c_void_p, c_int, c_int, c_int, c_int,
                                 c_float, c_int, c_void_p],
    "muse_groupnorm_nchunk": [c_int],
    "muse_avgpool2x2_nhwc": [c_void_p, c_void_p, c_int, c_int, c_int, c_int, c_int, c_void_p],
    "muse_avgpool2x2_nhwc_stats": [c_void_p, c_void_p, c_void_p, c_int, c_int, c_int, c_int, c_int, c_void_p],
    "muse_nchw_to_nhwc": [c_void_p, c_void_p, c_int, c_int, c_int, c_int, c_int, c_void_p],
    "muse_nhwc_to_nchw": [c_void_p, c_int, c_void_p, c_int, c_int, c_int, c_int, c_void_p],
    "muse_argmin_rows": [c_void_p, c_void_p, c_i64, c_int, c_i64, c_void_p],
    "muse_row_sumsq": [c_void_p, c_void_p, c_i64, c_int, c_i64, c_void_p],
    "muse_gather_rows": [c_void_p, c_void_p, c_void_p, c_int, c_i64, c_int, c_void_p],
    "muse_norm_res_fwd": [c_void_p, c_void_p, c_void_p, c_void_p, c_void_p, c_i64, c_int, c_float, c_int, c_void_p],
    "muse_adaln_fwd": [c_void_p, c_void_p, c_void_p, c_int, c_i64, c_int, c_void_p],
    "muse_adaln_fwd_ex": [c_void_p, c_void_p, c_void_p, c_void_p, c_int, c_i64, c_int, c_void_p],
    "muse_silu_fwd": [c_void_p, c_void_p, c_i64, c_void_p],
    "muse_dwconv3x3_nhwc": [c_void_p, c_void_p, c_void_p, c_int, c_int, c_int, c_int, c_void_p],
    "muse_space_to_depth2_nhwc": [c_void_p, c_void_p, c_int, c_int, c_int, c_int, c_int, c_void_p],
    "muse_grn_fwd": [c_void_p, c_void_p, c_void_p, c_void_p, c_void_p, c_int, c_i64, c_int, c_void_p],
    "muse_grn_fwd_ex": [c_void_p, c_void_p, c_void_p, c_void_p, c_void_p, c_void_p, c_int, c_i64, c_int, c_void_p],
    "muse_sinusoidal_encode": [c_void_p, c_void_p, c_i64, c_int, c_float, c_void_p],
    "muse_weighted_mean": [c_void_p, c_void_p, c_void_p, c_i64, c_void_p],
    "muse_norm_res_bwd_nblk": [c_i64],
    "muse_norm_res_bwd": [c_void_p, c_void_p, c_void_p, c_void_p, c_void_p, c_void_p, c_i64, c_int, c_float, c_int, c_void_p],
    "muse_norm_res_bwd_ex": [c_void_p, c_void_p, c_void_p, c_void_p, c_void_p, c_void_p, c_void_p, c_i64, c_int, c_float, c_int, c_void_p],
    "muse_adaln_bwd": [c_void_p, c_void_p, c_void_p, c_void_p, c_void_p, c_int, c_i64, c_int, c_void_p],
    "muse_norm_adaln_fwd": [c_void_p] * 7 + [c_int, c_i64, c_int, c_float, c_int, c_void_p],
    "muse_norm_adaln_bwd": [c_void_p] * 9 + [c_int, c_i64, c_int, c_float, c_int, c_void_p],
    "muse_norm_adaln_fwd_x3": [c_void_p] * 7 + [c_int, c_i64, c_int, c_float, c_int, *_IMG, c_void_p],
    "muse_norm_adaln_bwd_x3": [c_void_p] * 9 + [c_int, c_i64, c_int, c_float, c_int, *_IMG, c_void_p],
    "muse_colsum_segments": [c_void_p, c_void_p, c_int, c_int, c_int, c_void_p],
    "muse_silu_bwd": [c_void_p, c_void_p, c_void_p, c_i64, c_void_p],
    "muse_dwconv3x3_bwd_nchunk": [c_i64],
    "muse_dwconv3x3_bwd": [c_void_p, c_void_p, c_void_p, c_void_p, c_void_p, c_int, c_int, c_int, c_int, c_void_p],
    "muse_grn_bwd": [c_void_p, c_void_p, c_void_p, c_void_p, c_void_p, c_void_p, c_int, c_i64, c_int, c_void_p],
    "muse_scale_rows": [c_void_p, c_void_p, c_void_p, c_void_p, c_i64, c_int, c_i64, c_void_p],
    "muse_probe_tr16": [c_void_p, c_void_p, c_void_p],
}
_RESTYPES = {"muse_embed_bwd_scratch_floats": c_i64, "muse_embed_bwd2_scratch_bytes": c_i64}


class MuseHipError(RuntimeError):
    pass


def lib():
    global _lib
    if _lib is None:
        if not os.path.exists(LIB_PATH):
            raise MuseHipError(
                f"{LIB_PATH} not found: build it with `python __graft_entry__.py` (or `make -C open-muse_amd/csrc`). "
                "This package has no CPU / eager fallback.")
        handle = C.CDLL(LIB_PATH)
        for name, argtypes in SIGNATURES.items():
            fn = getattr(handle, name)
            fn.argtypes = argtypes
            fn.restype = _RESTYPES.get(name, C.c_int)
        _lib = handle
    return _lib


def check(code: int, what: str) -> None:
    if code != 0:
        raise MuseHipError(f"{what} failed with code {code} "
                           f"({'hipError' if code > 0 else {-1: 'bad argument', -2: 'alignment', -3: 'unsupported'}.get(code, '?')})")


def stream() -> int:
    return torch.cuda.current_stream().cuda_stream


def dt(t: torch.Tensor) -> int:
    if t.dtype == torch.float32:
        return F32
    if t.dtype == torch.bfloat16:
        return BF16
    raise MuseHipError(f"unsupported dtype {t.dtype}")


def ptr(t):
    return None if t is None else t.data_ptr()


def require_gpu(*tensors):
    for t in tensors:
        if t is not None and not t.is_cuda:
            raise MuseHipError("muse (MI355X build): tensors must live on the GPU; there is no CPU compute path")
```

### open-muse_amd/muse/modeling_maskgit_vqgan.py

```python
from __future__ import annotations

import math
import os
from typing import Tuple

import torch
import torch.nn.functional as F
from torch import nn

from . import ops
from ._hip import MuseHipError
from .modeling_utils import ConfigMixin, ModelMixin, register_to_config


class _Conv(nn.Module):
    def __init__(self, cin, cout, k, bias):
        super().__init__()
        self.weight = nn.Parameter(torch.empty(cout, cin, k, k))
        self.bias = nn.Parameter(torch.empty(cout)) if bias else None
        nn.init.kaiming_uniform_(self.weight, a=math.sqrt(5))
        if bias:
            bound = 1.0 / math.sqrt(cin * k * k)
            nn.init.uniform_(self.bias, -bound, bound)


class _GNInput:
    __slots__ = ("x", "scale", "shift")

    def __init__(self, x, scale, shift):
        self.x, self.scale, self.shift = x, scale, shift


class _Norm(nn.Module):
    def __init__(self, c):
        super().__init__()
        self.weight = nn.Parameter(torch.ones(c))
        self.bias = nn.Parameter(torch.zeros(c))


class _Res(nn.Module):
    def __init__(self, cin, cout):
        super().__init__()
        self.norm1 = _Norm(cin)
        self.conv1 = _Conv(cin, cout, 3, False)
        self.norm2 = _Norm(cout)
        self.conv2 = _Conv(cout, cout, 3, False)
        if cin != cout:
            self.nin_shortcut = _Conv(cout, cout, 1, False)


class _Down(nn.Module):
    def __init__(self, cin, cout, nb):
        super().__init__()
        self.block = nn.ModuleList([_Res(cin if i == 0 else cout, cout) for i in range(nb)])


class _Up(nn.Module):
    def __init__(self, cin, cout, nb, upsample):
        super().__init__()
        self.block = nn.ModuleList([_Res(cin if i == 0 else cout, cout) for i in range(nb)])
        if upsample:
            self.upsample_conv = _Conv(cout, cout, 3, True)


class _Encoder(nn.Module):
    def __init__(self, cfg):
        super().__init__()
        hc, mult, nb = cfg.hidden_channels, tuple(cfg.channel_mult), cfg.num_res_blocks
        self.conv_in = _Conv(cfg.num_channels, hc, 3, False)
        in_mult = (1,) + mult
        self.down = nn.ModuleList([_Down(hc * in_mult[i], hc * mult[i], nb) for i in range(len(mult))])
        mid = hc * mult[-1]
        self.mid = nn.ModuleList([_Res(mid, mid) for _ in range(nb)])
        self.norm_out = _Norm(mid)
        self.conv_out = _Conv(mid, cfg.z_channels, 1, True)


class _Decoder(nn.Module):
    def __init__(self, cfg):
        super().__init__()
        hc, mult, nb = cfg.hidden_channels, tuple(cfg.channel_mult), cfg.num_res_blocks
        nres = len(mult)
        mid = hc * mult[-1]
        self.conv_in = _Conv(cfg.z_channels, mid, 3, True)
        self.mid = nn.ModuleList([_Res(mid, mid) for _ in range(nb)])
        ups = []
        for lvl in range(nres):
            cin = hc * mult[-1] if lvl == nres - 1 else hc * mult[lvl + 1]
            ups.append(_Up(cin, hc * mult[lvl], nb, lvl != 0))
        self.up = nn.ModuleList(ups)
        self.norm_out = _Norm(hc * mult[0])
        self.conv_out = _Conv(hc * mult[0], cfg.num_channels, 3, True)


class _Quantizer(nn.Module):
    def __init__(self, n, d):
        super().__init__()
        self.embedding = nn.Embedding(n, d)
        self.embedding.weight.data.uniform_(-1.0 / n, 1.0 / n)


class _ConvEngine:

    def _init_engine(self):
        self.compute_dtype = torch.float32
        self.fuse_gn_stats = True
        self.fuse_gn_apply = os.environ.get("MUSE_GN_FUSE", "1") != "0"
        self.direct_conv_in = os.environ.get("MUSE_CONV_IN_DIRECT", "1") != "0"
        self.conv_in_nchw = os.environ.get("MUSE_CONV_IN_NCHW", "1") != "0"
        self.fuse_pool = os.environ.get("MUSE_POOL_FUSE", "1") != "0"
        self.dma_conv = True
        self.direct_conv_out = os.environ.get("MUSE_CONV_OUT_DIRECT", "1") != "0"
        self.upsample_split = os.environ.get("MUSE_UPSAMPLE_SPLIT", "1") != "0"
        self._packed = {}

    def _check(self, t):
        if not t.is_cuda:
            raise MuseHipError(f"{type(self).__name__} (MI355X build) has no CPU path: move the model and inputs to the GPU")

    def set_compute_dtype(self, dtype):
        if dtype not in (torch.float32, torch.bfloat16, "bf16x3"):
            raise ValueError('compute dtype must be torch.float32, torch.bfloat16 or "bf16x3"')
        self.compute_dtype = dtype
        return self

    def _act_dtype(self):
        return torch.bfloat16 if self.compute_dtype == torch.bfloat16 else torch.float32

    def _apply(self, fn, recurse=True):
        self._packed = {}
        return super()._apply(fn, recurse)

    def load_state_dict(self, state_dict, strict: bool = True, assign: bool = False):
        self._packed = {}
        return super().load_state_dict(state_dict, strict=strict, assign=assign)

    def _cpad(self, c, cd):
        q = 4 if cd == torch.float32 else 8
        return (c + q - 1) // q * q

    def _w(self, conv: _Conv, cd):
        key = (id(conv), cd)
        hit = self._packed.get(key)
        if hit is None:
            w = conv.weight.data
            cout, cin, k, _ = w.shape
            cp = self._cpad(cin, cd)
            wp = torch.zeros((cout, k, k, cp), dtype=torch.float32, device=w.device)
            wp[..., :cin] = w.permute(0, 2, 3, 1)
            wp = wp.contiguous()
            if cd == torch.bfloat16:
                wp = ops.cast_to_bf16(wp)
            elif cd == "bf16x3":
                wp = ops.split_bf16(wp)
            hit = (wp, cp, cout, k, None if conv.bias is None else conv.bias.data.float().contiguous())
            self._packed[key] = hit
        return hit

    def _conv_in_image(self, pixel_values, conv, B, H, W, cd):
        C = pixel_values.shape[1]
        cout, cin, k, _ = conv.weight.shape
        cpad = self._cpad(C, cd)
        x = pixel_values.float()
        if (cd == "bf16x3" and self.direct_conv_in and self.conv_in_nchw and cin == C and ops.conv_in_direct_ok(cin, cout, k, cpad, W)):
            w4, bias = self._w_conv_in_direct(conv)
            return ops.conv_in_direct_nchw(x.contiguous(), w4, B, H, W, cin, cout, bias=bias, gn_groups=32 if self.fuse_gn_stats else 0)
        return self._conv_in(ops.nchw_to_nhwc(x, self._act_dtype(), cpad), conv, B, H, W, cd, cpad)

    def _w_conv_in_direct(self, conv):
        cout, cin, k, _ = conv.weight.shape
        key = (id(conv), "direct")
        hit = self._packed.get(key)
        if hit is None:
            w4 = torch.zeros((cout, 9, 4), dtype=torch.float32, device=conv.weight.device)
            w4[:, :, :cin] = conv.weight.data.float().permute(0, 2, 3, 1).reshape(cout, 9, cin)
            hit = (w4.contiguous(), None if conv.bias is None else conv.bias.data.float().contiguous())
            self._packed[key] = hit
        return hit

    def _conv_in(self, x, conv, B, H, W, cd, cpad):
        cout, cin, k, _ = conv.weight.shape
        if cd == "bf16x3" and self.direct_conv_in and ops.conv_in_direct_ok(cin, cout, k, cpad, W):
            hit = self._w_conv_in_direct(conv)
            return ops.conv_in_direct(x, hit[0], B, H, W, cin, cpad, cout, bias=hit[1], gn_groups=32 if self.fuse_gn_stats else 0)
        return self._conv(x, conv, B, H, W, cd, gn_next=True)

    def _conv(self, x, conv, B, H, W, cd, residual=None, upsample=False, gn_next=False, pool=False):
        wp, cp, cout, k, bias = self._w(conv, cd)
        if pool:
            return ops.conv2d_nhwc_gn_split2_pool(x.x, x.scale, x.shift, wp[0], wp[1], B, H, W, cp, cout, bias=bias, residual=residual,
                                                  gn_groups=32 if (gn_next and self.fuse_gn_stats) else 0)
        if isinstance(x, _GNInput):
            return ops.conv2d_nhwc_gn_split2(x.x, x.scale, x.shift, wp[0], wp[1], B, H, W, cp, cout, bias=bias, residual=residual,
                                             gn_groups=32 if (gn_next and self.fuse_gn_stats) else 0)
        if isinstance(x, tuple):
            return ops.conv2d_nhwc_split2(x[0], x[1], wp[0], wp[1], B, H, W, cp, cout, bias=bias, residual=residual,
                                          gn_groups=32 if (gn_next and self.fuse_gn_stats) else 0)
        if cd == "bf16x3":
            if (self.dma_conv and self.upsample_split and not upsample and k == 3 and x.dtype == torch.float32 and x.is_contiguous()
                    and cp == x.shape[-1] and ops.conv_split2_ok(B, H, W, cp, cout, k) and ops.conv_slab_ok(H, W, cp)):
                hi, lo = ops.split_f32(x)
                return ops.conv2d_nhwc_split2(hi, lo, wp[0], wp[1], B, H, W, cp, cout, bias=bias, residual=residual,
                                              gn_groups=32 if (gn_next and self.fuse_gn_stats) else 0)
            return ops.conv2d_nhwc_split(x, wp[0], wp[1], B, H, W, cp, cout, k, bias=bias, residual=residual, upsample=upsample,
                                         gn_groups=32 if (gn_next and self.fuse_gn_stats) else 0)
        return ops.conv2d_nhwc(x, wp, B, H, W, cp, cout, k, bias=bias, residual=residual, upsample=upsample)

    def _pool_ok(self, x, conv: _Conv, B, H, W, cd):
        cout, cin, k, _ = conv.weight.shape
        return (cd == "bf16x3" and self.fuse_pool and isinstance(x, _GNInput) and cin == cout
                and ops.conv_gn_split2_pool_ok(B, H, W, cin, cout, k, 32 if self.fuse_gn_stats else 0))

    def _upsample_conv(self, h, conv: _Conv, B, H, W, cd):
        cout, cin, k, _ = conv.weight.shape
        if (cd == "bf16x3" and self.dma_conv and self.upsample_split and cin % 8 == 0 and h.dtype == torch.float32
                and ops.conv_split2_ok(B, H, W, cin, cout, k)):
            planes = ops.upsample2x_split(h, B, H // 2, W // 2, cin)
            return self._conv(planes, conv, B, H, W, cd, gn_next=True)
        return self._conv(h, conv, B, H, W, cd, upsample=True, gn_next=True)

    def _conv_out(self, h, norm: _Norm, conv: _Conv, B, H, W, cd):
        cout, cin, k, _ = conv.weight.shape
        stats = getattr(h, "_gn_stats", None)
        if (cd == "bf16x3" and self.direct_conv_out and stats is not None and h.dtype == torch.float32
                and ops.conv_out_direct_ok(H, W, cin, cout, k)):
            key = (id(conv), "direct_out")
            hit = self._packed.get(key)
            if hit is None:
                hit = (conv.weight.data.float().permute(0, 2, 3, 1).reshape(cout, 9, cin).contiguous(),
                       None if conv.bias is None else conv.bias.data.float().contiguous())
                self._packed[key] = hit
            sc, sh = ops.groupnorm_scale_shift(stats, norm.weight.data, norm.bias.data, B, H * W, cin, groups=32, eps=1e-6)
            return ops.conv_out_direct(h, sc, sh, hit[0], hit[1], B, H, W, cin, cout)
        return self._conv(self._gn_for(h, norm, conv, B, H, W, cd), conv, B, H, W, cd)

    def _gn(self, x, norm: _Norm, B, HW, C, silu=True):
        return ops.groupnorm_silu_nhwc(x, norm.weight.data, norm.bias.data, B, HW, C, groups=32, eps=1e-6, silu=silu)

    def _gn_for(self, x, norm: _Norm, conv: _Conv, B, H, W, cd):
        cout, cin, k, _ = conv.weight.shape
        stats = getattr(x, "_gn_stats", None)
        if (cd == "bf16x3" and self.dma_conv and self.fuse_gn_apply and stats is not None and ops.conv_slab_ok(H, W, cin)
                and ops.conv_gn_split2_ok(B, H, W, cin, cout, k)):
            sc, sh = ops.groupnorm_scale_shift(stats, norm.weight.data, norm.bias.data, B, H * W, cin, groups=32, eps=1e-6)
            return _GNInput(x, sc, sh)
        if cd == "bf16x3" and self.dma_conv and ops.conv_split2_ok(B, H, W, cin, cout, k) and (256 % (cin // 4)) == 0:
            return ops.groupnorm_silu_nhwc_split(x, norm.weight.data, norm.bias.data, B, H * W, cin, groups=32, eps=1e-6, silu=True,
                                                 stats=getattr(x, "_gn_stats", None))
        return self._gn(x, norm, B, H * W, cin)


class MaskGitVQGAN(_ConvEngine, ModelMixin, ConfigMixin):
    _cast_selects_compute_mode = True

    def _compute_mode_for(self, dtype):
        if dtype is None or not dtype.is_floating_point:
            return False
        self.set_compute_dtype("bf16x3" if dtype in (torch.float16, torch.bfloat16) else torch.float32)
        return True

    @register_to_config
    def __init__(
        self,
        resolution: int = 256,
        num_channels: int = 3,
        hidden_channels: int = 128,
        channel_mult: Tuple = (1, 1, 2, 2, 4),
        num_res_blocks: int = 2,
        attn_resolutions: int = (16,),
        z_channels: int = 256,
        num_embeddings: int = 1024,
        quantized_embed_dim: int = 256,
        dropout: float = 0.0,
        resample_with_conv: bool = True,
        commitment_cost: float = 0.25,
    ):
        super().__init__()
        if dropout != 0.0:
            raise NotImplementedError("dropout > 0 in the VQGAN is outside the MI355X hot-path build")
        if z_channels != quantized_embed_dim:
            raise ValueError("z_channels must equal quantized_embed_dim")
        self.config.num_resolutions = len(channel_mult)
        self.config.reduction_factor = 2 ** (self.config.num_resolutions - 1)
        self.config.latent_size = resolution // self.config.reduction_factor
        self.encoder = _Encoder(self.config)
        self.decoder = _Decoder(self.config)
        self.quantize = _Quantizer(num_embeddings, quantized_embed_dim)
        self._init_engine()

    def _res(self, x, blk: _Res, B, H, W, cd, pool=False):
        cin = blk.conv1.weight.shape[1]
        cout = blk.conv1.weight.shape[0]
        h = self._conv(self._gn_for(x, blk.norm1, blk.conv1, B, H, W, cd), blk.conv1, B, H, W, cd, gn_next=True)
        if cin == cout:
            g = self._gn_for(h, blk.norm2, blk.conv2, B, H, W, cd)
            if pool and self._pool_ok(g, blk.conv2, B, H, W, cd):
                out = self._conv(g, blk.conv2, B, H, W, cd, residual=x, gn_next=True, pool=True)
                out._pooled = True
                return out
            return self._conv(g, blk.conv2, B, H, W, cd, residual=x, gn_next=True)
        h = self._conv(self._gn_for(h, blk.norm2, blk.conv2, B, H, W, cd), blk.conv2, B, H, W, cd)
        return self._conv(h, blk.nin_shortcut, B, H, W, cd, residual=h, gn_next=True)

    @torch.no_grad()
    def _encode_nhwc(self, pixel_values):
        self._check(pixel_values)
        cd = self.compute_dtype
        enc = self.encoder
        B, C, H, W = pixel_values.shape
        h = self._conv_in_image(pixel_values, enc.conv_in, B, H, W, cd)
        nres = self.config.num_resolutions
        for lvl, down in enumerate(enc.down):
            for i, blk in enumerate(down.block):
                h = self._res(h, blk, B, H, W, cd, pool=lvl != nres - 1 and i == len(down.block) - 1)
            if lvl != nres - 1:
                if not getattr(h, "_pooled", False):
                    h = ops.avgpool2x2_nhwc(h, B, H, W, h.shape[-1], gn_groups=32 if (cd == "bf16x3" and self.fuse_gn_stats) else 0)
                H, W = H // 2, W // 2
        for blk in enc.mid:
            h = self._res(h, blk, B, H, W, cd)
        h = self._gn_for(h, enc.norm_out, enc.conv_out, B, H, W, cd)
        z = self._conv(h, enc.conv_out, B, H, W, cd)
        z = z.view(B * H * W, -1)
        if z.dtype != torch.float32:
            z = ops.cast_to_f32(z)
        return z, (B, H, W)

    @torch.no_grad()
    def _decode_nhwc(self, zq, B, H, W):
        cd = self.compute_dtype
        dec = self.decoder
        nres = self.config.num_resolutions
        h = self._conv(zq, dec.conv_in, B, H, W, cd, gn_next=True)
        for blk in dec.mid:
            h = self._res(h, blk, B, H, W, cd)
        for lvl in reversed(range(nres)):
            up = dec.up[lvl]
            for blk in up.block:
                h = self._res(h, blk, B, H, W, cd)
            if lvl != 0:
                H, W = H * 2, W * 2
                h = self._upsample_conv(h, up.upsample_conv, B, H, W, cd)
        out = self._conv_out(h, dec.norm_out, dec.conv_out, B, H, W, cd)
        return ops.nhwc_to_nchw(out, self.config.num_channels)

    def _codebook(self):
        return self.quantize.embedding.weight.data

    @torch.no_grad()
    def encode(self, pixel_values, return_loss=False):
        z, (B, H, W) = self._encode_nhwc(pixel_values)
        cb = self._codebook()
        idx = ops.vq_nearest(z, cb)
        zq_rows = ops.gather_rows(cb, idx, torch.float32)
        zq = ops.nhwc_to_nchw(zq_rows.view(B, H, W, -1), zq_rows.shape[1])
        out = (zq, idx.view(B, H * W))
        if return_loss:
            zc = ops.nhwc_to_nchw(z.view(B, H, W, -1), z.shape[1])
            mse = torch.mean((zq - zc) ** 2)
            out = out + (mse + self.config.commitment_cost * mse,)
        return out

    @torch.no_grad()
    def decode(self, quantized_states):
        self._check(quantized_states)
        B, C, H, W = quantized_states.shape
        cd = self.compute_dtype
        zq = ops.nchw_to_nhwc(quantized_states.float(), self._act_dtype(), C)
        return self._decode_nhwc(zq, B, H, W)

    @torch.no_grad()
    def decode_code(self, codebook_indices):
        self._check(codebook_indices)
        B, T = codebook_indices.shape
        side = int(math.sqrt(T))
        zq = ops.gather_rows(self._codebook(), codebook_indices.contiguous().view(-1), self._act_dtype())
        return self._decode_nhwc(zq.view(B, side, side, -1), B, side, side)

    @torch.no_grad()
    def get_code(self, pixel_values):
        z, (B, H, W) = self._encode_nhwc(pixel_values)
        return ops.vq_nearest(z, self._codebook()).view(B, H * W)

    @torch.no_grad()
    def get_soft_code(self, pixel_values, temp=1.0, stochastic=False):
        z, (B, H, W) = self._encode_nhwc(pixel_values)
        cb = self._codebook()
        soft = ops.vq_neg_distances_scaled(z, cb, 1.0 / float(temp))
        ops.softmax_(soft, soft.shape[0], soft.shape[1], soft.shape[1])
        code = torch.multinomial(soft, 1) if stochastic else ops.vq_nearest(z, cb)
        return soft.view(B, H * W, -1), code.view(B, H * W)

    def forward(self, pixel_values, return_loss=False):
        enc = self.encode(pixel_values, return_loss)
        rec = self.decode(enc[0])
        out = (rec, enc[0], enc[1])
        if return_loss:
            out = out + (enc[2],)
        return out
```

### open-muse_amd/muse/modeling_taming_vqgan.py

```python
from __future__ import annotations

import math
from types import SimpleNamespace
from typing import Tuple

import torch
import torch.nn.functional as F
from torch import nn

from . import ops
from .modeling_maskgit_vqgan import _Conv, _ConvEngine, _Norm, _Quantizer
from .modeling_utils import ConfigMixin, ModelMixin, register_to_config


class _Res(nn.Module):
    def __init__(self, cin, cout):
        super().__init__()
        self.norm1 = _Norm(cin)
        self.conv1 = _Conv(cin, cout, 3, True)
        self.norm2 = _Norm(cout)
        self.conv2 = _Conv(cout, cout, 3, True)
        if cin != cout:
            self.nin_shortcut = _Conv(cin, cout, 1, True)

# ... 56 lines not shown
        super().__init__()
        hc, mult, nb = cfg.hidden_channels, tuple(cfg.channel_mult), cfg.num_res_blocks
        nres, attn_res = len(mult), tuple(cfg.attn_resolutions)
        mid = hc * mult[-1]
        self.conv_in = _Conv(cfg.z_channels, mid, 3, True)
        self.mid = _Mid(mid, cfg.no_attn_mid_block)
        cur, levels = cfg.resolution // 2 ** (nres - 1), [None] * nres
        for i in reversed(range(nres)):
            cin = mid if i == nres - 1 else hc * mult[i + 1]
            levels[i] = _Level(cin, hc * mult[i], nb + 1, cur in attn_res, "upsample" if i != 0 else None, cfg.resample_with_conv)
            if i != 0:
                cur *= 2
        self.up = nn.ModuleList(levels)
        self.norm_out = _Norm(hc * mult[0])
        self.conv_out = _Conv(hc * mult[0], cfg.num_channels, 3, True)


class VQGANModel(_ConvEngine, ModelMixin, ConfigMixin):
    _cast_selects_compute_mode = True

    def _compute_mode_for(self, dtype):
        if dtype is None or not dtype.is_floating_point:
            return False
        self.set_compute_dtype("bf16x3" if dtype in (torch.float16, torch.bfloat16) else torch.float32)
        return True

    @register_to_config
    def __init__(
        self,
        resolution: int = 256,
        num_channels: int = 3,
        hidden_channels: int = 128,
        channel_mult: Tuple = (1, 1, 2, 2, 4),
        num_res_blocks: int = 2,
        attn_resolutions: int = (16,),
        no_attn_mid_block: bool = False,
        z_channels: int = 256,
        num_embeddings: int = 1024,
        quantized_embed_dim: int = 256,
        dropout: float = 0.0,
        resample_with_conv: bool = True,
        commitment_cost: float = 0.25,
    ):
        super().__init__()
        if dropout != 0.0:
            raise NotImplementedError("dropout > 0 in the VQGAN is outside the MI355X hot-path build (frozen tokenizer)")
        self.config.num_resolutions = len(channel_mult)
        self.config.reduction_factor = 2 ** (self.config.num_resolutions - 1)
        self.config.latent_size = resolution // self.config.reduction_factor
        self.encoder = _Encoder(self.config)
        self.decoder = _Decoder(self.config)
        self.quantize = _Quantizer(num_embeddings, quantized_embed_dim)
        self.quant_conv = _Conv(z_channels, quantized_embed_dim, 1, True)
        self.post_quant_conv = _Conv(quantized_embed_dim, z_channels, 1, True)
        self._init_engine()

    @property
    def num_embeddings(self):
        return self.config.num_embeddings

    def _res(self, x, blk: _Res, B, H, W, cd):
        h = self._conv(self._gn_for(x, blk.norm1, blk.conv1, B, H, W, cd), blk.conv1, B, H, W, cd, gn_next=True)
        sc = self._conv(x, blk.nin_shortcut, B, H, W, cd) if hasattr(blk, "nin_shortcut") else x
        return self._conv(self._gn_for(h, blk.norm2, blk.conv2, B, H, W, cd), blk.conv2, B, H, W, cd, residual=sc, gn_next=True)

    def _qkv(self, att: _Attn, cd):
        key = (id(att), "qkv")
        hit = self._packed.get(key)
        if hit is None:
            hit = SimpleNamespace(weight=torch.cat([att.q.weight.data, att.k.weight.data, att.v.weight.data], 0),
                                  bias=torch.cat([att.q.bias.data, att.k.bias.data, att.v.bias.data], 0))
            self._packed[key] = hit
        return hit

    def _attn(self, x, att: _Attn, B, H, W, cd):
        C, HW = att.norm.weight.shape[0], H * W
        h = self._gn(x, att.norm, B, HW, C, silu=False)
        qkv = self._conv(h, self._qkv(att, cd), B, H, W, cd).view(B * HW, 3 * C)
        scores = torch.empty((B, HW, HW), dtype=torch.float32, device=x.device)
        ops.gemm(qkv, qkv, scores, HW, HW, C, la=0, lb=0, lda=3 * C, ldb=3 * C, ldc=HW, b_off=C, alpha=float(int(C) ** -0.5),
                 batch=B, sA=(HW * 3 * C, 0), sB=(HW * 3 * C, 0), sC=(HW * HW, 0))
        ops.softmax_(scores, B * HW, HW, HW)
        probs = scores if qkv.dtype == torch.float32 else ops.cast_to_bf16(scores)
        ctx = torch.empty((B, H, W, C), dtype=qkv.dtype, device=x.device)
        ops.gemm(probs, qkv, ctx, HW, C, HW, la=0, lb=1, lda=HW, ldb=3 * C, ldc=C, b_off=2 * C, batch=B,
                 sA=(HW * HW, 0), sB=(HW * 3 * C, 0), sC=(HW * C, 0))
        return self._conv(ctx, att.proj_out, B, H, W, cd, residual=x, gn_next=True)

    def _level(self, x, lvl: _Level, B, H, W, cd):
        run_attn = len(lvl.attn) > 1
        for i, blk in enumerate(lvl.block):
            x = self._res(x, blk, B, H, W, cd)
            if run_attn:
                x = self._attn(x, lvl.attn[i], B, H, W, cd)
        return x

    def _mid(self, x, mid: _Mid, B, H, W, cd):
        x = self._res(x, mid.block_1, B, H, W, cd)
        if hasattr(mid, "attn_1"):
            x = self._attn(x, mid.attn_1, B, H, W, cd)
        return self._res(x, mid.block_2, B, H, W, cd)

    @torch.no_grad()
    def _encode_nhwc(self, pixel_values):
        self._check(pixel_values)
        cd, enc = self.compute_dtype, self.encoder
        B, C, H, W = pixel_values.shape
        if (H | W) % (1 << (self.config.num_resolutions - 1)):
            raise ValueError("image height / width must be multiples of the reduction factor")
        x = ops.nchw_to_nhwc(pixel_values.float(), self._act_dtype(), self._cpad(C, cd))
        h = self._conv_in(x, enc.conv_in, B, H, W, cd, self._cpad(C, cd))
        for lvl in enc.down:
            h = self._level(h, lvl, B, H, W, cd)
            if hasattr(lvl, "downsample"):
                H, W = H // 2, W // 2
                if hasattr(lvl.downsample, "conv"):
                    h = self._conv(h, lvl.downsample.conv, B, H, W, cd, upsample=2, gn_next=True)
                else:
                    h = ops.avgpool2x2_nhwc(h, B, 2 * H, 2 * W, h.shape[-1], gn_groups=32 if (cd == "bf16x3" and self.fuse_gn_stats) else 0)
        h = self._mid(h, enc.mid, B, H, W, cd)
        h = self._conv(self._gn_for(h, enc.norm_out, enc.conv_out, B, H, W, cd), enc.conv_out, B, H, W, cd)
        z = self._conv(h, self.quant_conv, B, H, W, cd).view(B * H * W, -1)
        if z.dtype != torch.float32:
            z = ops.cast_to_f32(z)
        return z, (B, H, W)

    @torch.no_grad()
    def _decode_nhwc(self, zq, B, H, W):
        cd, dec = self.compute_dtype, self.decoder
        h = self._conv(zq, self.post_quant_conv, B, H, W, cd)
        h = self._conv(h, dec.conv_in, B, H, W, cd, gn_next=True)
        h = self._mid(h, dec.mid, B, H, W, cd)
        for lvl in reversed(dec.up):
            h = self._level(h, lvl, B, H, W, cd)
            if hasattr(lvl, "upsample"):
                H, W = H * 2, W * 2
                if hasattr(lvl.upsample, "conv"):
                    h = self._upsample_conv(h, lvl.upsample.conv, B, H, W, cd)
                else:
                    if h.shape[-1] % (8 if h.dtype == torch.bfloat16 else 4) == 0:
                        h = ops.upsample2x(h.contiguous(), B, H // 2, W // 2, h.shape[-1])
                    else:
                        h = F.interpolate(h.permute(0, 3, 1, 2), scale_factor=2.0, mode="nearest").permute(0, 2, 3, 1).contiguous()
        h = self._conv_out(h, dec.norm_out, dec.conv_out, B, H, W, cd)
        return ops.nhwc_to_nchw(h, self.config.num_channels)

    def _codebook(self):
        return self.quantize.embedding.weight.data

    @torch.no_grad()
    def encode(self, pixel_values, return_loss=False):
        z, (B, H, W) = self._encode_nhwc(pixel_values)
        cb = self._codebook()
        idx = ops.vq_nearest(z, cb)
        zq_rows = ops.gather_rows(cb, idx, torch.float32)
        zq = ops.nhwc_to_nchw(zq_rows.view(B, H, W, -1), zq_rows.shape[1])
        out = (zq, idx.view(B, H * W))
        if return_loss:
            zc = ops.nhwc_to_nchw(z.view(B, H, W, -1), z.shape[1])
            mse = torch.mean((zq - zc) ** 2)
            out = out + (mse + self.config.commitment_cost * mse,)
        return out

    @torch.no_grad()
    def decode(self, quantized_states):
        self._check(quantized_states)
        B, C, H, W = quantized_states.shape
        zq = ops.nchw_to_nhwc(quantized_states.float(), self._act_dtype(), C)
        return self._decode_nhwc(zq, B, H, W)

    @torch.no_grad()
    def decode_code(self, codebook_indices):
        self._check(codebook_indices)
        B, T = codebook_indices.shape
        side = int(math.sqrt(T))
        zq = ops.gather_rows(self._codebook(), codebook_indices.contiguous().view(-1), self._act_dtype())
        return self._decode_nhwc(zq.view(B, side, side, -1), B, side, side)

    @torch.no_grad()
    def get_code(self, pixel_values):
        z, (B, H, W) = self._encode_nhwc(pixel_values)
        return ops.vq_nearest(z, self._codebook()).view(B, H * W)

    @torch.no_grad()
    def get_soft_code(self, pixel_values, temp=1.0, stochastic=False):
        z, (B, H, W) = self._encode_nhwc(pixel_values)
        cb = self._codebook()
        dist = torch.cdist(z, cb).pow(2)
        soft = F.softmax(-dist / temp, dim=-1)
        code = torch.multinomial(soft, 1) if stochastic else ops.vq_nearest(z, cb)
        return soft.view(B, H * W, -1), code.view(B, H * W)

    def forward(self, pixel_values, return_loss=False):
        enc = self.encode(pixel_values, return_loss)
        rec = self.decode(enc[0])
        out = (rec, enc[0], enc[1])
        if return_loss:
            out = out + (enc[2],)
        return out
```

### open-muse_amd/muse/ops.py

```python
from __future__ import annotations

import ctypes as C
import math
import os
import weakref

import torch

from . import _hip
from ._hip import BF16, F16, F32, GemmDesc, check, dt, lib, ptr, require_gpu, stream

USE_TR = os.environ.get("MUSE_GEMM_TR", "1") != "0"


def _esz(t):
    return t.element_size()


_PROF = None


PROF_BYTES = {}


# ... 1420 lines not shown


def gradnorm_finalize(slab, chunk_first, num_tensors, psum, grad_scale, max_norm, out):
    require_gpu(slab, chunk_first, psum, out)
    check(lib().muse_gradnorm_finalize(slab.data_ptr(), chunk_first.data_ptr(), int(num_tensors), psum.data_ptr(), float(grad_scale),
                                       float(max_norm), out.data_ptr(), stream()), "muse_gradnorm_finalize")


def grad_scale_flat_(g, scale):
    require_gpu(g, scale)
    check(lib().muse_grad_scale_flat(g.data_ptr(), g.numel(), scale.data_ptr(), stream()), "muse_grad_scale_flat")


def grad_scale_multi_(table, chunk_first, num_tensors, num_chunks, scale):
    require_gpu(table, chunk_first, scale)
    check(lib().muse_grad_scale_multi(table.data_ptr(), int(table.shape[1]), chunk_first.data_ptr(), int(num_tensors), int(num_chunks),
                                      scale.data_ptr(), stream()), "muse_grad_scale_multi")


def cast_to_bf16(src, dst=None):
    require_gpu(src)
    if dst is None:
        dst = torch.empty(src.shape, dtype=torch.bfloat16, device=src.device)
    check(lib().muse_cast_f32_to_bf16(src.data_ptr(), dst.data_ptr(), src.numel(), stream()), "muse_cast_f32_to_bf16")
    return dst


def cast_to_f32(src, dst=None):
    require_gpu(src)
    given = dst is not None
    if dst is None:
        dst = torch.empty(src.shape, dtype=torch.float32, device=src.device)
    check(lib().muse_cast_bf16_to_f32(src.data_ptr(), dst.data_ptr(), src.numel(), stream()), "muse_cast_bf16_to_f32")
    return _touched(dst) if given else dst


def mask_sample(tokens, class_ids, timesteps, noise, mask_id, codebook_size, min_masking_rate=0.0):
    require_gpu(tokens, class_ids, timesteps, noise)
    B, S = tokens.shape
    input_ids = torch.empty((B, S + 1), dtype=torch.int64, device=tokens.device)
    labels = torch.empty((B, S + 1), dtype=torch.int64, device=tokens.device)
    mask_prob = torch.empty(B, dtype=torch.float32, device=tokens.device)
    check(lib().muse_mask_sample(tokens.data_ptr(), class_ids.data_ptr(), timesteps.data_ptr(), noise.data_ptr(),
                                 input_ids.data_ptr(), labels.data_ptr(), mask_prob.data_ptr(), B, S, mask_id, codebook_size,
                                 min_masking_rate, stream()), "muse_mask_sample")
    return input_ids, labels, mask_prob


def sample_step(cond_logits, input_ids, mask_id, vocab, temperature, sched_mask_len, *, uncond_logits=None, guidance_scale=0.0,
                noise_exp=None, noise_u=None, seed=0, step=0, want_raw=False):
    require_gpu(cond_logits, input_ids)
    B, S = input_ids.shape

    def layout(t):
        if t.dim() != 3 or t.shape[0] != B or t.shape[1] != S or t.stride(2) != 1 or t.dtype != torch.float32 or t.shape[2] < vocab:
            raise _hip.MuseHipError("sample_step: logits must be a float32 [B, S, >= vocab] view with a contiguous last dim")
        return t.stride(0), t.stride(1)

    lay = layout(cond_logits)
    if uncond_logits is not None and layout(uncond_logits) != lay:
        raise _hip.MuseHipError("sample_step: cond / uncond logits must share a layout")
    ids = input_ids.contiguous()
    sampled, nxt = torch.empty_like(ids), torch.empty_like(ids)
    raw = torch.empty_like(ids) if want_raw else None
    conf = torch.empty(B * S, dtype=torch.float32, device=ids.device)
    if noise_exp is not None:
        noise_exp = noise_exp.reshape(B * S, vocab).to(device=ids.device, dtype=torch.float32).contiguous()
    if noise_u is not None:
        noise_u = noise_u.reshape(B * S).to(device=ids.device, dtype=torch.float32).contiguous()
    check(lib().muse_sample_step(cond_logits.data_ptr(), ptr(uncond_logits), float(guidance_scale), lay[0], lay[1], int(vocab),
                                 ids.data_ptr(), int(mask_id), ptr(noise_exp), ptr(noise_u), int(seed) & (2 ** 64 - 1), int(step),
                                 float(temperature), int(sched_mask_len), B, S, ptr(raw), sampled.data_ptr(), nxt.data_ptr(),
                                 conf.data_ptr(), stream()), "muse_sample_step")
    return sampled, nxt, raw


def mask_tokens(tokens, mask_id, *, timesteps=None, mask_prob=None, noise=None, rects=None, min_masking_rate=0.0, all_labels=False,
                want_weight=False, weight_min=0.3):
    require_gpu(tokens)
    B, S = tokens.shape
    dev = tokens.device
    tokens = tokens.contiguous()
    input_ids, labels = torch.empty_like(tokens), torch.empty_like(tokens)
    lw = torch.empty((B, S), dtype=torch.float32, device=dev) if want_weight else None
    mp = torch.empty(B, dtype=torch.float32, device=dev)
    f = lambda t: None if t is None else t.to(device=dev, dtype=torch.float32).contiguous()
    timesteps, mask_prob, noise = f(timesteps), f(mask_prob), f(noise)
    if rects is not None:
        rects = rects.to(device=dev, dtype=torch.int32).contiguous()
    check(lib().muse_mask_tokens(tokens.data_ptr(), ptr(timesteps), ptr(mask_prob), ptr(noise), ptr(rects), input_ids.data_ptr(),
                                 labels.data_ptr(), ptr(lw), mp.data_ptr(), B, S, int(mask_id), float(min_masking_rate),
                                 1 if all_labels else 0, float(weight_min), stream()), "muse_mask_tokens")
    return input_ids, labels, lw, mp


def dropout(x, p, seed, offset, out=None):
    require_gpu(x)
    if not x.is_contiguous():
        raise _hip.MuseHipError("dropout expects a contiguous tensor")
    y = out if out is not None else torch.empty_like(x)
    check(lib().muse_dropout(x.data_ptr(), y.data_ptr(), dt(x), x.numel(), float(p), int(seed) & (2 ** 64 - 1), int(offset) & (2 ** 64 - 1),
                             stream()), "muse_dropout")
    return _touched(y) if out is not None else y


def cond_dropout(x, empty, uniforms, prob):
    require_gpu(x, empty, uniforms)
    B = x.shape[0]
    xc = x.float().contiguous()
    per = xc.numel() // B
    e = empty.float().contiguous()
    if e.numel() != per:
        raise _hip.MuseHipError("cond_dropout: the empty embedding must have the shape of one batch element")
    out = torch.empty_like(xc)
    check(lib().muse_cond_dropout(xc.data_ptr(), e.data_ptr(), uniforms.float().contiguous().data_ptr(), out.data_ptr(), B, per,
                                  float(prob), stream()), "muse_cond_dropout")
    return out


def conv2d_nhwc(x, w, B, H, W, Cin, Cout, KS, bias=None, residual=None, upsample=False):
    require_gpu(x, w)
    out = torch.empty((B, H, W, Cout), dtype=x.dtype, device=x.device)
    e0 = _prof_begin()
    check(lib().muse_conv2d_nhwc(x.data_ptr(), w.data_ptr(), ptr(bias), ptr(residual), out.data_ptr(), dt(x), B, H, W, Cin,
                                 Cout, KS, int(upsample), stream()), "muse_conv2d_nhwc")
    _prof_end(e0, f"conv_{'bf16' if x.dtype == torch.bfloat16 else 'f32'}", 2.0 * B * H * W * Cout * KS * KS * Cin)
    return out


def split_bf16(w):
    hi = cast_to_bf16(w.contiguous())
    lo = cast_to_bf16((w - cast_to_f32(hi)).contiguous())
    return hi, lo


def conv2d_nhwc_split(x, w_hi, w_lo, B, H, W, Cin, Cout, KS, bias=None, residual=None, upsample=False, gn_groups=0):
    require_gpu(x, w_hi, w_lo)
    out = torch.empty((B, H, W, Cout), dtype=torch.float32, device=x.device)
    part, nchunk = None, 0
    cpg = Cout // gn_groups if gn_groups else 0
    if gn_groups and Cout % gn_groups == 0 and cpg in (4, 8, 16, 32) and (H * W) % 128 == 0:
        nchunk = (H * W) // 128
        part = torch.empty(B * nchunk * gn_groups * 2, dtype=torch.float64, device=out.device)
    e0 = _prof_begin()
    check(lib().muse_conv2d_nhwc_split(x.data_ptr(), w_hi.data_ptr(), w_lo.data_ptr(), ptr(bias), ptr(residual), out.data_ptr(),
                                       ptr(part), gn_groups if part is not None else 0, B, H, W, Cin, Cout, KS,
                                       int(upsample), stream()), "muse_conv2d_nhwc_split")
    _prof_end(e0, "conv_bf16x3", 2.0 * B * H * W * Cout * KS * KS * Cin)
    if part is not None:
        out._gn_stats = (part, nchunk)
    return out


def conv2d_nhwc_split2(x_hi, x_lo, w_hi, w_lo, B, H, W, Cin, Cout, bias=None, residual=None, gn_groups=0):
    require_gpu(x_hi, x_lo, w_hi, w_lo)
    out = torch.empty((B, H, W, Cout), dtype=torch.float32, device=x_hi.device)
    part, nchunk = None, 0
    if gn_groups and conv_gn_stats_ok(H, W, Cout, gn_groups):
        nchunk = (H * W) // 256
        part = torch.empty(B * nchunk * gn_groups * 2, dtype=torch.float64, device=out.device)
    e0 = _prof_begin()
    check(lib().muse_conv2d_nhwc_split2(x_hi.data_ptr(), x_lo.data_ptr(), w_hi.data_ptr(), w_lo.data_ptr(), ptr(bias),
                                        ptr(residual), out.data_ptr(), ptr(part), gn_groups if part is not None else 0,
                                        B, H, W, Cin, Cout, 3, stream()), "muse_conv2d_nhwc_split2")
    _prof_end(e0, "conv_bf16x3_dma", 2.0 * B * H * W * Cout * 9 * Cin)
    if e0 is not None:
        PROF_BYTES["conv_bf16x3_dma"] = PROF_BYTES.get("conv_bf16x3_dma", 0.0) + _nbytes(x_hi, x_lo, w_hi, w_lo, residual, out)
    if part is not None:
        out._gn_stats = (part, nchunk)
    return out


def conv_in_direct_ok(Cin, Cout, KS, Cpad, W=256):
    return (KS == 3 and Cin <= 4 and Cpad % 4 == 0 and Cpad >= 4 and Cout % 4 == 0 and Cout // 4 <= 256 and 256 % (Cout // 4) == 0
            and W <= 1022)


def conv_in_direct(x, w4, B, H, W, Cin, Cpad, Cout, bias=None, gn_groups=0):
    require_gpu(x, w4)
    out = torch.empty((B, H, W, Cout), dtype=torch.float32, device=x.device)
    part = None
    if gn_groups and gn_groups * 4 == Cout:
        part = torch.empty(B * H * gn_groups * 2, dtype=torch.float64, device=x.device)
    e0 = _prof_begin()
    check(lib().muse_conv_in_direct(x.data_ptr(), w4.data_ptr(), ptr(bias), out.data_ptr(), ptr(part), gn_groups if part is not None else 0,
                                    B, H, W, Cin, Cpad, Cout, stream()), "muse_conv_in_direct")
    _prof_end(e0, "conv_in_direct", _nbytes(x, out), "byte")
    if part is not None:
        out._gn_stats = (part, H)
    return out


def conv_in_direct_nchw(x, w4, B, H, W, Cin, Cout, bias=None, gn_groups=0):
    require_gpu(x, w4)
    if x.dtype != torch.float32 or not x.is_contiguous() or tuple(x.shape) != (B, Cin, H, W):
        raise ValueError("conv_in_direct_nchw: x must be a contiguous f32 [B, Cin, H, W] tensor")
    out = torch.empty((B, H, W, Cout), dtype=torch.float32, device=x.device)
    part = None
    if gn_groups and gn_groups * 4 == Cout:
        part = torch.empty(B * H * gn_groups * 2, dtype=torch.float64, device=x.device)
    e0 = _prof_begin()
    check(lib().muse_conv_in_direct_nchw(x.data_ptr(), w4.data_ptr(), ptr(bias), out.data_ptr(), ptr(part), gn_groups if part is not None else 0,
                                         B, H, W, Cin, Cout, stream()), "muse_conv_in_direct_nchw")
    _prof_end(e0, "conv_in_direct", _nbytes(x, out), "byte")
    if part is not None:
        out._gn_stats = (part, H)
    return out


def conv_out_direct_ok(H, W, Cin, Cout, KS):
    return KS == 3 and Cout <= 4 and Cin % 32 == 0 and Cin >= 32 and H % 16 == 0 and W % 16 == 0


def conv_out_direct(x, scale, shift, w, bias, B, H, W, Cin, Cout):
    require_gpu(x, scale, shift, w)
    out = torch.empty((B, H, W, Cout), dtype=torch.float32, device=x.device)
    e0 = _prof_begin()
    check(lib().muse_conv_out_direct(x.data_ptr(), scale.data_ptr(), shift.data_ptr(), w.data_ptr(), ptr(bias), out.data_ptr(),
                                     B, H, W, Cin, Cout, stream()), "muse_conv_out_direct")
    _prof_end(e0, "conv_out_direct", _nbytes(x, out), "byte")
    return out


def upsample2x(x, B, H, W, C):
    require_gpu(x)
    y = torch.empty((B, 2 * H, 2 * W, C), dtype=x.dtype, device=x.device)
    check(lib().muse_upsample2x_nhwc(x.data_ptr(), y.data_ptr(), dt(x), B, H, W, C, stream()), "muse_upsample2x_nhwc")
    return y


def upsample2x_split(x, B, H, W, C):
    require_gpu(x)
    hi = torch.empty((B, 2 * H, 2 * W, C), dtype=torch.bfloat16, device=x.device)
    lo = torch.empty_like(hi)
    e0 = _prof_begin()
    check(lib().muse_upsample2x_split_nhwc(x.data_ptr(), hi.data_ptr(), lo.data_ptr(), B, H, W, C, stream()), "muse_upsample2x_split_nhwc")
    _prof_end(e0, "upsample2x_split", _nbytes(x, hi, lo), "byte")
    return hi, lo


_CONV_PERSISTENT = [os.environ.get("MUSE_CONV_PERSIST", "1") != "0"]


class conv_persistent:

    def __init__(self, on):
        self.on = bool(on)

    def __enter__(self):
        self.prev = _CONV_PERSISTENT[0]
        _CONV_PERSISTENT[0] = self.on
        return self

    def __exit__(self, *exc):
        _CONV_PERSISTENT[0] = self.prev
        return False


def conv_gn_split2_ok(B, H, W, Cin, Cout, KS):
    return bool(lib().muse_conv2d_nhwc_gn_split2_ok(B, H, W, Cin, Cout, KS))


def groupnorm_scale_shift(stats, gamma, beta, B, HW, C, groups=32, eps=1e-6):
    part, nchunk = stats
    require_gpu(part, gamma, beta)
    sc = torch.empty((B, C), dtype=torch.float32, device=part.device)
    sh = torch.empty((B, C), dtype=torch.float32, device=part.device)
    check(lib().muse_groupnorm_scale_shift(part.data_ptr(), nchunk, gamma.data_ptr(), beta.data_ptr(), sc.data_ptr(), sh.data_ptr(),
                                           B, HW, C, groups, eps, stream()), "muse_groupnorm_scale_shift")
    return sc, sh


def conv2d_nhwc_gn_split2(x, scale, shift, w_hi, w_lo, B, H, W, Cin, Cout, bias=None, residual=None, gn_groups=0):
    require_gpu(x, scale, shift, w_hi, w_lo)
    out = torch.empty((B, H, W, Cout), dtype=torch.float32, device=x.device)
    part, nchunk = None, 0
    if gn_groups and conv_gn_stats_ok(H, W, Cout, gn_groups):
        nchunk = (H * W) // 256
        part = torch.empty(B * nchunk * gn_groups * 2, dtype=torch.float64, device=out.device)
    e0 = _prof_begin()
    check(lib().muse_conv2d_nhwc_gn_split2(x.data_ptr(), scale.data_ptr(), shift.data_ptr(), w_hi.data_ptr(), w_lo.data_ptr(), ptr(bias),
                                           ptr(residual), out.data_ptr(), ptr(part), gn_groups if part is not None else 0,
                                           B, H, W, Cin, Cout, 3, int(_CONV_PERSISTENT[0]), stream()), "muse_conv2d_nhwc_gn_split2")
    _prof_end(e0, "conv_bf16x3_dma", 2.0 * B * H * W * Cout * 9 * Cin)
    if e0 is not None:
        PROF_BYTES["conv_bf16x3_dma"] = PROF_BYTES.get("conv_bf16x3_dma", 0.0) + _nbytes(x, w_hi, w_lo, residual, out)
    if part is not None:
        out._gn_stats = (part, nchunk)
    return out


def conv_gn_split2_pool_ok(B, H, W, Cin, Cout, KS, gn_groups=0):
    return conv_gn_split2_ok(B, H, W, Cin, Cout, KS) and (not gn_groups or conv_gn_stats_ok(H, W, Cout, gn_groups))


def conv2d_nhwc_gn_split2_pool(x, scale, shift, w_hi, w_lo, B, H, W, Cin, Cout, bias=None, residual=None, gn_groups=0):
    require_gpu(x, scale, shift, w_hi, w_lo)
    out = torch.empty((B, H // 2, W // 2, Cout), dtype=torch.float32, device=x.device)
    part, nchunk = None, 0
    if gn_groups and conv_gn_stats_ok(H, W, Cout, gn_groups):
        nchunk = (H * W) // 256
        part = torch.empty(B * nchunk * gn_groups * 2, dtype=torch.float64, device=out.device)
    e0 = _prof_begin()
    check(lib().muse_conv2d_nhwc_gn_split2_pool(x.data_ptr(), scale.data_ptr(), shift.data_ptr(), w_hi.data_ptr(), w_lo.data_ptr(), ptr(bias),
                                                ptr(residual), out.data_ptr(), ptr(part), gn_groups if part is not None else 0,
                                                B, H, W, Cin, Cout, 3, int(_CONV_PERSISTENT[0]), stream()), "muse_conv2d_nhwc_gn_split2_pool")
    _prof_end(e0, "conv_bf16x3_dma", 2.0 * B * H * W * Cout * 9 * Cin)
    if e0 is not None:
        PROF_BYTES["conv_bf16x3_dma"] = PROF_BYTES.get("conv_bf16x3_dma", 0.0) + _nbytes(x, w_hi, w_lo, residual, out)
    if part is not None:
        out._gn_stats = (part, nchunk)
    return out


def conv_split2_ok(B, H, W, Cin, Cout, KS):
    M = B * H * W
    return KS == 3 and Cin % 32 == 0 and Cout % 4 == 0 and M * Cin * 2 < (1 << 32) - 64 and M < (1 << 31) - 256


def conv_slab_ok(H, W, Cin):
    import os
    return H % 16 == 0 and W % 16 == 0 and Cin % 64 == 0 and os.environ.get("MUSE_CONV_SLAB", "1") != "0"


def conv_gn_stats_ok(H, W, Cout, groups):
    cpg = Cout // groups if groups else 0
    return groups in (32, 64) and Cout % groups == 0 and (H * W) % 256 == 0 and 4 <= cpg <= 128 and (cpg & (cpg - 1)) == 0


def groupnorm_silu_nhwc_split(x, gamma, beta, B, HW, C, groups=32, eps=1e-6, silu=True, stats=None):
    require_gpu(x, gamma, beta)
    hi = torch.empty(x.shape, dtype=torch.bfloat16, device=x.device)
    lo = torch.empty(x.shape, dtype=torch.bfloat16, device=x.device)
    if stats is not None:
        part, snc = stats
    else:
        nchunk = lib().muse_groupnorm_nchunk(HW)
        part, snc = torch.empty(B * nchunk * groups * 2, dtype=torch.float64, device=x.device), 0
    e0 = _prof_begin()
    check(lib().muse_groupnorm_silu_nhwc_split(x.data_ptr(), hi.data_ptr(), lo.data_ptr(), gamma.data_ptr(), beta.data_ptr(),
                                               part.data_ptr(), snc, B, HW, C, groups, eps, 1 if silu else 0, stream()),
          "muse_groupnorm_silu_nhwc_split")
    _prof_end(e0, "groupnorm_silu", _nbytes(x, hi, lo), "byte")
    return hi, lo


def groupnorm_silu_nhwc(x, gamma, beta, B, HW, C, groups=32, eps=1e-6, silu=True):
    require_gpu(x, gamma, beta)
    y = torch.empty_like(x)
    nchunk = lib().muse_groupnorm_nchunk(HW)
    part = torch.empty(B * nchunk * groups * 2, dtype=torch.float64, device=x.device)
    e0 = _prof_begin()
    check(lib().muse_groupnorm_silu_nhwc(x.data_ptr(), y.data_ptr(), dt(x), gamma.data_ptr(), beta.data_ptr(), part.data_ptr(),
                                         B, HW, C, groups, eps, 1 if silu else 0, stream()), "muse_groupnorm_silu_nhwc")
    _prof_end(e0, "groupnorm_silu", _nbytes(x, y), "byte")
    return y


def avgpool2x2_nhwc(x, B, H, W, C_, gn_groups=0):
    require_gpu(x)
    y = torch.empty((B, H // 2, W // 2, C_), dtype=x.dtype, device=x.device)
    e0 = _prof_begin()
    vpp = C_ // 4
    if gn_groups and x.dtype == torch.float32 and C_ % 4 == 0 and C_ % gn_groups == 0 and vpp <= 256 and 256 % vpp == 0:
        nchunk = lib().muse_groupnorm_nchunk((H // 2) * (W // 2))
        part = torch.empty(B * nchunk * gn_groups * 2, dtype=torch.float64, device=x.device)
        check(lib().muse_avgpool2x2_nhwc_stats(x.data_ptr(), y.data_ptr(), part.data_ptr(), gn_groups, B, H, W, C_, stream()),
              "muse_avgpool2x2_nhwc_stats")
        y._gn_stats = (part, nchunk)
    else:
        check(lib().muse_avgpool2x2_nhwc(x.data_ptr(), y.data_ptr(), dt(x), B, H, W, C_, stream()), "muse_avgpool2x2_nhwc")
    _prof_end(e0, "avgpool2x2", _nbytes(x, y), "byte")
    return y


def nchw_to_nhwc(x, out_dtype, cpad):
    require_gpu(x)
    B, C_, H, W = x.shape
    x = x.contiguous()
    out = torch.empty((B, H, W, cpad), dtype=out_dtype, device=x.device)
    check(lib().muse_nchw_to_nhwc(x.data_ptr(), out.data_ptr(), dt(out), B, C_, H * W, cpad, stream()), "muse_nchw_to_nhwc")
    return out


def nhwc_to_nchw(x, C_):
    require_gpu(x)
    B, H, W, cpad = x.shape
    out = torch.empty((B, C_, H, W), dtype=torch.float32, device=x.device)
    check(lib().muse_nhwc_to_nchw(x.data_ptr(), dt(x), out.data_ptr(), B, C_, H * W, cpad, stream()), "muse_nhwc_to_nchw")
    return out


def vq_nearest(z_flat, codebook, en=None, return_dist=False):
    require_gpu(z_flat, codebook)
    N, D = z_flat.shape
    Kc = codebook.shape[0]
    zn = torch.empty(N, dtype=torch.float32, device=z_flat.device)
    check(lib().muse_row_sumsq(z_flat.data_ptr(), zn.data_ptr(), N, D, z_flat.stride(0), stream()), "muse_row_sumsq")
    if en is None:
        en = torch.empty(Kc, dtype=torch.float32, device=z_flat.device)
        check(lib().muse_row_sumsq(codebook.data_ptr(), en.data_ptr(), Kc, D, codebook.stride(0), stream()), "muse_row_sumsq")
    dist = torch.empty((N, Kc), dtype=torch.float32, device=z_flat.device)
    gemm(z_flat, codebook, dist, N, Kc, D, la=0, lb=0, lda=z_flat.stride(0), ldb=codebook.stride(0), ldc=Kc, alpha=-2.0,
         bias=en, rowvec=zn)
    idx = torch.empty(N, dtype=torch.int64, device=z_flat.device)
    check(lib().muse_argmin_rows(dist.data_ptr(), idx.data_ptr(), N, Kc, Kc, stream()), "muse_argmin_rows")
    return (idx, dist) if return_dist else idx


def vq_neg_distances_scaled(z_flat, codebook, inv_temp):
    require_gpu(z_flat, codebook)
    N, D = z_flat.shape
    Kc = codebook.shape[0]
    zn = torch.empty(N, dtype=torch.float32, device=z_flat.device)
    en = torch.empty(Kc, dtype=torch.float32, device=z_flat.device)
    check(lib().muse_row_sumsq(z_flat.data_ptr(), zn.data_ptr(), N, D, z_flat.stride(0), stream()), "muse_row_sumsq")
    check(lib().muse_row_sumsq(codebook.data_ptr(), en.data_ptr(), Kc, D, codebook.stride(0), stream()), "muse_row_sumsq")
    out = torch.empty((N, Kc), dtype=torch.float32, device=z_flat.device)
    gemm(z_flat, codebook, out, N, Kc, D, la=0, lb=0, lda=z_flat.stride(0), ldb=codebook.stride(0), ldc=Kc, alpha=2.0 * inv_temp,
         bias=en.mul_(-inv_temp), rowvec=zn.mul_(-inv_temp))
    return out


def gather_rows(table, idx, out_dtype):
    require_gpu(table, idx)
    rows = idx.numel()
    cols = table.shape[1]
    out = torch.empty((rows, cols), dtype=out_dtype, device=table.device)
    check(lib().muse_gather_rows(table.data_ptr(), idx.data_ptr(), out.data_ptr(), dt(out), rows, cols, stream()), "muse_gather_rows")
    return out


def norm_res_fwd(x, w, eps, mode, residual=None, want_pre=False):
    require_gpu(x)
    rows, cols = x.shape
    y = torch.empty_like(x)
    pre = torch.empty_like(x) if want_pre else None
    check(lib().muse_norm_res_fwd(x.data_ptr(), ptr(residual), ptr(w), y.data_ptr(), ptr(pre), rows, cols, eps, mode, stream()),
          "muse_norm_res_fwd")
    return y, pre


def adaln_fwd(x, ss, batch, out_dtype=torch.float32):
    require_gpu(x, ss)
    rows, C_ = x.shape
    y = torch.empty((rows, C_), dtype=out_dtype, device=x.device)
    f32 = out_dtype == torch.float32
    check(lib().muse_adaln_fwd_ex(x.data_ptr(), ss.data_ptr(), y.data_ptr() if f32 else None, None if f32 else y.data_ptr(), batch,
                                  rows // batch, C_, stream()), "muse_adaln_fwd_ex")
    return y


def silu_fwd(x):
    require_gpu(x)
    y = torch.empty_like(x)
    check(lib().muse_silu_fwd(x.data_ptr(), y.data_ptr(), x.numel(), stream()), "muse_silu_fwd")
    return y


def dwconv3x3_nhwc(x, w, B, H, W, C_):
    require_gpu(x, w)
    y = torch.empty_like(x)
    check(lib().muse_dwconv3x3_nhwc(x.data_ptr(), w.data_ptr(), y.data_ptr(), B, H, W, C_, stream()), "muse_dwconv3x3_nhwc")
    return y


def space_to_depth2(x, B, H, W, C_):
    require_gpu(x)
    y = torch.empty((B * (H // 2) * (W // 2), 4 * C_), dtype=torch.float32, device=x.device)
    check(lib().muse_space_to_depth2_nhwc(x.data_ptr(), y.data_ptr(), B, H, W, C_, 0, stream()), "muse_space_to_depth2_nhwc")
    return y


def depth_to_space2(x, B, H, W, C_):
    require_gpu(x)
    y = torch.empty((B * H * W, C_), dtype=torch.float32, device=x.device)
    check(lib().muse_space_to_depth2_nhwc(x.data_ptr(), y.data_ptr(), B, H, W, C_, 1, stream()), "muse_space_to_depth2_nhwc")
    return y


def grn_fwd(x, gamma, beta, B, S, want_stats=False, out_dtype=torch.float32):
    require_gpu(x, gamma, beta)
    C_ = x.shape[1]
    bf = out_dtype == torch.bfloat16 and C_ % 4 == 0
    y = torch.empty(x.shape, dtype=torch.bfloat16 if bf else torch.float32, device=x.device)
    stats = torch.empty(2 * B * C_, dtype=torch.float32, device=x.device)
    check(lib().muse_grn_fwd_ex(x.data_ptr(), gamma.data_ptr(), beta.data_ptr(), None if bf else y.data_ptr(), y.data_ptr() if bf else None,
                                stats.data_ptr(), B, S, C_, stream()), "muse_grn_fwd_ex")
    return (y, stats) if want_stats else y


def sinusoidal_encode(features, dim, max_positions=10000.0):
    require_gpu(features)
    f = features.reshape(-1).float().contiguous()
    out = torch.empty((f.numel(), dim), dtype=torch.float32, device=f.device)
    check(lib().muse_sinusoidal_encode(f.data_ptr(), out.data_ptr(), f.numel(), dim, max_positions, stream()), "muse_sinusoidal_encode")
    return out


def weighted_mean(v, w):
    require_gpu(v, w)
    out = torch.empty(1, dtype=torch.float32, device=v.device)
    check(lib().muse_weighted_mean(v.data_ptr(), w.data_ptr(), out.data_ptr(), v.numel(), stream()), "muse_weighted_mean")
    return out


def colsum(part, out, accumulate=False):
    require_gpu(part, out)
    rows, cols = part.shape
    check(lib().muse_colsum(part.data_ptr(), out.data_ptr(), rows, cols, 1 if accumulate else 0, stream()), "muse_colsum")
    return out


def add_rowvec_(x, b):
    require_gpu(x, b)
    if x.dtype != torch.float32 or b.dtype != torch.float32 or not x.is_contiguous():
        raise _hip.MuseHipError("add_rowvec_: contiguous f32 rows and an f32 vector")
    check(lib().muse_add_rowvec(x.data_ptr(), b.data_ptr(), x.numel() // x.shape[-1], x.shape[-1], stream()), "muse_add_rowvec")
    return _touched(x)


def bias_grad(dy, cols=None):
    require_gpu(dy)
    rows = dy.shape[0]
    cols = dy.shape[1] if cols is None else cols
    if dy.stride(1) != 1:
        raise _hip.MuseHipError("bias_grad: unit column stride")
    R = lib().muse_bias_grad_rows_per_block()
    part = torch.empty(((rows + R - 1) // R, cols), dtype=torch.float32, device=dy.device)
    check(lib().muse_bias_grad_partial(dy.data_ptr(), dt(dy), part.data_ptr(), rows, cols, dy.stride(0), stream()), "muse_bias_grad_partial")
    return colsum(part, torch.empty(cols, dtype=torch.float32, device=dy.device))


def norm_res_bwd(dy, v, w, eps, mode, dpre=None, want_dw=True, also_bf16=False):
    require_gpu(dy, v)
    rows, cols = v.shape
    dv = torch.empty_like(v)
    dvb = torch.empty(v.shape, dtype=torch.bfloat16, device=v.device) if also_bf16 else None
    nblk = lib().muse_norm_res_bwd_nblk(rows)
    part = torch.empty((nblk, cols), dtype=torch.float32, device=v.device)
    check(lib().muse_norm_res_bwd_ex(dy.data_ptr(), ptr(dpre), v.data_ptr(), ptr(w), dv.data_ptr(), ptr(dvb), part.data_ptr(), rows,
                                     cols, eps, mode, stream()), "muse_norm_res_bwd_ex")
    dw = colsum(part, torch.empty(cols, dtype=torch.float32, device=v.device)) if want_dw else None
    return (dv, dw, dvb) if also_bf16 else (dv, dw)


def norm_adaln_ok(rows, cols, batch):
    return cols % 4 == 0 and cols <= 1024 and rows % batch == 0 and (rows // batch) % 16 == 0

# ... 103 lines not shown
```

Baseline: 1234 images/s.

## Add dedicated bf16x3 1x1 conv kernel and fused VQ nearest-code search

Result: no change. 1236 images/s (median of 4 runs) (+0.2%).

```diff
diff --git a/include/muse_hip.h b/include/muse_hip.h
--- a/include/muse_hip.h
+++ b/include/muse_hip.h
@@ -208,6 +208,10 @@
 int muse_conv2d_nhwc_split(const float* in, const void* w_hi, const void* w_lo, const float* bias, const float* residual,
                            float* out, double* gn_partial, int32_t gn_groups, int32_t batch, int32_t H, int32_t W,
                            int32_t Cin, int32_t Cout, int32_t KS, int32_t upsample, void* stream);
+int muse_conv1x1_nhwc_split_ok(int32_t batch, int32_t H, int32_t W, int32_t Cin, int32_t Cout);
+int muse_conv1x1_nhwc_split(const float* in, const void* w_hi, const void* w_lo, const float* bias, const float* residual,
+                            float* out, double* gn_partial, int32_t gn_groups, int32_t batch, int32_t H, int32_t W,
+                            int32_t Cin, int32_t Cout, void* stream);
 int muse_conv2d_nhwc_split2(const void* in_hi, const void* in_lo, const void* w_hi, const void* w_lo, const float* bias,
                             const float* residual, float* out, double* gn_partial, int32_t gn_groups, int32_t batch,
                             int32_t H, int32_t W, int32_t Cin, int32_t Cout, int32_t KS, void* stream);
@@ -247,6 +251,9 @@
                       void* stream);
 int muse_argmin_rows(const float* dist, int64_t* idx, int64_t rows, int32_t ncodes, int64_t ld, void* stream);
 int muse_row_sumsq(const float* x, float* out, int64_t rows, int32_t cols, int64_t ld, void* stream);
+int muse_vq_nearest_ok(int64_t rows, int32_t ncodes, int32_t dim, int64_t ldz, int64_t ldc);
+int muse_vq_nearest(const float* z, const float* codebook, const float* zn, const float* en, int64_t* idx, int64_t rows, int32_t ncodes,
+                    int32_t dim, int64_t ldz, int64_t ldc, void* stream);
 int muse_gather_rows(const float* table, const int64_t* idx, void* out, int32_t out_dtype, int64_t rows, int32_t cols,
                      void* stream);
 
diff --git a/open-muse_amd/csrc/conv_split.hip b/open-muse_amd/csrc/conv_split.hip
--- a/open-muse_amd/csrc/conv_split.hip
+++ b/open-muse_amd/csrc/conv_split.hip
@@ -191,3 +191,201 @@
   hipLaunchKernelGGL(conv_split_kernel, dim3(ntm * ntn), dim3(256), lds, (hipStream_t)stream, sp);
   return (int)hipGetLastError();
 }
+
+namespace c1x1 {
+constexpr int BK = 64, IMG = 128 * 160;
+constexpr int CST = 128 * 4 + 16;
+constexpr int RED_OFF = 128 * CST;
+constexpr int LDS = RED_OFF + 4 * 32 * 2 * 8 > 4 * IMG ? RED_OFF + 4 * 32 * 2 * 8 : 4 * IMG;
+static_assert(RED_OFF + 4 * 32 * 2 * 8 <= 4 * IMG, "C staging + reduction scratch live inside the operand stages");
+struct Params {
+  const float* x; const void* w_hi; const void* w_lo; const float* bias; const float* residual; float* out;
+  double* gn_partial;
+  int gn_groups, gn_cpg;
+  int M, N, K, HW;
+  int nper;
+};
+}
+
+__global__ __launch_bounds__(256, 2) void conv1x1_split_kernel(c1x1::Params q) {
+  using namespace c1x1;
+  extern __shared__ __attribute__((aligned(16))) unsigned char smem[];
+  unsigned char* tAh = smem;
+  unsigned char* tAl = smem + IMG;
+  unsigned char* tBh = smem + 2 * IMG;
+  unsigned char* tBl = smem + 3 * IMG;
+
+  const int ntm = (q.M + 127) >> 7, ntn = (q.N + 127) >> 7, nsplit = (ntn + q.nper - 1) / q.nper, nwg = ntm * nsplit;
+  const int bq = nwg >> 3, br = nwg & 7, xcd = blockIdx.x & 7, bi = blockIdx.x >> 3;
+  const int wid = (xcd < br ? xcd * (bq + 1) : br * (bq + 1) + (xcd - br) * bq) + bi;
+  const int m0 = (wid / nsplit) << 7, nt0 = (wid % nsplit) * q.nper, nt1 = min(ntn, nt0 + q.nper);
+  const int rows = min(128, q.M - m0);
+
+  using ALoader = PlainLoader<float, 0, 128, 256>;
+  using BLoader = PlainLoader<bf16_t, 0, 128, 256>;
+  const GemmParams unused{};
+  ALoader la; la.init(q.x + (long)m0 * q.K, q.K, rows, q.K, 0, unused);
+  BLoader lh; lh.init(q.w_hi, q.K, q.N, q.K, 0, unused);
+  BLoader ll; ll.init(q.w_lo, q.K, q.N, q.K, 0, unused);
+  const unsigned tile_bytes = (unsigned)(128 * q.K * 2);
+
+  const int lane = threadIdx.x & 63, wave = threadIdx.x >> 6;
+  const int wr = (wave >> 1) * 64, wc = (wave & 1) * 64;
+  f32x4 acc[4][4];
+#pragma unroll
+  for (int i = 0; i < 4; ++i)
+#pragma unroll
+    for (int j = 0; j < 4; ++j) acc[i][j] = f32x4{0.f, 0.f, 0.f, 0.f};
+
+  u32x4 ra[ALoader::NCH], rh[BLoader::NCH], rl[BLoader::NCH];
+  const int nk = (q.K + BK - 1) / BK;
+
+  auto fetch = [&](int nt, int kt) {
+    const int k0 = kt * BK;
+#pragma unroll
+    for (int i = 0; i < ALoader::NCH; ++i) ra[i] = la.load(i, k0);
+#pragma unroll
+    for (int i = 0; i < BLoader::NCH; ++i) {
+      const int c = threadIdx.x + 256 * i;
+      const bool ok = (nt * 128 + c / BLoader::CPR) < q.N && (k0 + (c % BLoader::CPR) * 8) < q.K;
+      const unsigned off = ok ? lh.voff[i] + (unsigned)nt * tile_bytes : lh.oob;
+      rh[i] = buf_load16(lh.rs, off, (unsigned)k0 * 2u);
+      rl[i] = buf_load16(ll.rs, off, (unsigned)k0 * 2u);
+    }
+  };
+  auto stage = [&]() {
+#pragma unroll
+    for (int i = 0; i < ALoader::NCH; ++i) {
+      const int c = threadIdx.x + 256 * i;
+      const int off = (c >> 4) * 160 + (c & 15) * 8;
+      u32x2 hi, lo;
+      split4(ra[i], hi, lo);
+      *(u32x2*)(tAh + off) = hi;
+      *(u32x2*)(tAl + off) = lo;
+    }
+#pragma unroll
+    for (int i = 0; i < BLoader::NCH; ++i) {
+      *(u32x4*)(tBh + BLoader::lds_off(i)) = rh[i];
+      *(u32x4*)(tBl + BLoader::lds_off(i)) = rl[i];
+    }
+  };
+
+  fetch(nt0, 0);
+  stage();
+  __syncthreads();
+  for (int nt = nt0; nt < nt1; ++nt) {
+    for (int kt = 0; kt < nk; ++kt) {
+      const bool last_k = (kt + 1) == nk, more = !last_k || (nt + 1) < nt1;
+      if (more) fetch(last_k ? nt + 1 : nt, last_k ? 0 : kt + 1);
+#pragma unroll
+      for (int ks = 0; ks < 2; ++ks) {
+        bf16x8 ah[4], al[4];
+#pragma unroll
+        for (int i = 0; i < 4; ++i) {
+          ah[i] = frag_bf16<0, 128>(tAh, wr + i * 16, ks, lane);
+          al[i] = frag_bf16<0, 128>(tAl, wr + i * 16, ks, lane);
+        }
+#pragma unroll
+        for (int j = 0; j < 4; ++j) {
+          const bf16x8 bh = frag_bf16<0, 128>(tBh, wc + j * 16, ks, lane);
+          const bf16x8 bl = frag_bf16<0, 128>(tBl, wc + j * 16, ks, lane);
+#pragma unroll
+          for (int i = 0; i < 4; ++i) {
+            acc[i][j] = __builtin_amdgcn_mfma_f32_16x16x32_bf16(bl, ah[i], acc[i][j], 0, 0, 0);
+            acc[i][j] = __builtin_amdgcn_mfma_f32_16x16x32_bf16(bh, al[i], acc[i][j], 0, 0, 0);
+            acc[i][j] = __builtin_amdgcn_mfma_f32_16x16x32_bf16(bh, ah[i], acc[i][j], 0, 0, 0);
+          }
+        }
+      }
+      __syncthreads();
+      if (last_k) {
+        const int n0 = nt << 7;
+#pragma unroll
+        for (int i = 0; i < 4; ++i) {
+          const int ml = wr + i * 16 + (lane & 15);
+#pragma unroll
+          for (int j = 0; j < 4; ++j) {
+            const int nl = wc + j * 16 + 4 * (lane >> 4);
+            float v[4];
+#pragma unroll
+            for (int r = 0; r < 4; ++r) {
+              v[r] = acc[i][j][r] + ((q.bias && (n0 + nl + r) < q.N) ? q.bias[n0 + nl + r] : 0.f);
+              acc[i][j][r] = 0.f;
+            }
+            OutVec<float>::store4((float*)(smem + ml * CST) + nl, v);
+          }
+        }
+        __syncthreads();
+        double gs = 0.0, gq = 0.0;
+        const int col = (threadIdx.x & 31) * 4, n = n0 + col;
+#pragma unroll 4
+        for (int it = 0; it < 16; ++it) {
+          const int row = (threadIdx.x >> 5) + 8 * it;
+          if (row < rows && n < q.N) {
+            float v[4];
+            OutVec<float>::load4((const float*)(smem + row * CST) + col, v);
+            const long o = (long)(m0 + row) * q.N + n;
+            if (q.residual) { float t[4]; OutVec<float>::load4(q.residual + o, t); v[0] += t[0]; v[1] += t[1]; v[2] += t[2]; v[3] += t[3]; }
+            OutVec<float>::store4(q.out + o, v);
+#pragma unroll
+            for (int r = 0; r < 4; ++r) { gs += (double)v[r]; gq += (double)v[r] * (double)v[r]; }
+          }
+        }
+        double* red = (double*)(smem + RED_OFF);
+        if (q.gn_partial) {
+          gs += __shfl_xor(gs, 32, 64); gq += __shfl_xor(gq, 32, 64);
+          if (lane < 32) { red[(wave * 32 + lane) * 2] = gs; red[(wave * 32 + lane) * 2 + 1] = gq; }
+        }
+        __syncthreads();
+        if (q.gn_partial && threadIdx.x < 32) {
+          double cs = 0.0, cq = 0.0;
+#pragma unroll
+          for (int w = 0; w < 4; ++w) { cs += red[(w * 32 + threadIdx.x) * 2]; cq += red[(w * 32 + threadIdx.x) * 2 + 1]; }
+          const int cpc = q.gn_cpg >> 2;
+          for (int o = 1; o < cpc; o <<= 1) { cs += __shfl_xor(cs, o, 64); cq += __shfl_xor(cq, o, 64); }
+          if ((threadIdx.x & (cpc - 1)) == 0 && n < q.N) {
+            const int b = m0 / q.HW, chunk = (m0 - b * q.HW) >> 7, nchunk = q.HW >> 7;
+            double* o2 = q.gn_partial + (((long)b * nchunk + chunk) * q.gn_groups + n / q.gn_cpg) * 2;
+            o2[0] = cs; o2[1] = cq;
+          }
+        }
+        if (q.gn_partial) __syncthreads();
+      }
+      if (more) {
+        stage();
+        __syncthreads();
+      }
+    }
+  }
+}
+
+extern "C" int muse_conv1x1_nhwc_split_ok(int32_t batch, int32_t H, int32_t W, int32_t Cin, int32_t Cout) {
+  const int64_t M = (int64_t)batch * H * W;
+  if (batch < 1 || H < 1 || W < 1 || Cin < 8 || (Cin & 7) || Cout < 4 || (Cout & 3)) return 0;
+  if (M >= (1LL << 31) - 128 || ((M + 127) / 128) * ((Cout + 127) / 128) >= (1LL << 31)) return 0;
+  if ((int64_t)(Cout + 128) * Cin * 2 >= (1LL << 32) || (int64_t)128 * Cin * 4 >= (1LL << 32)) return 0;
+  return 1;
+}
+extern "C" int muse_conv1x1_nhwc_split(const float* in, const void* w_hi, const void* w_lo, const float* bias, const float* residual,
+                                       float* out, double* gn_partial, int32_t gn_groups, int32_t batch, int32_t H, int32_t W,
+                                       int32_t Cin, int32_t Cout, void* stream) {
+  if (!muse_conv1x1_nhwc_split_ok(batch, H, W, Cin, Cout)) return MUSE_ERR_UNSUPPORTED;
+  if ((((uintptr_t)in) & 15) || (((uintptr_t)w_hi) & 15) || (((uintptr_t)w_lo) & 15) || (((uintptr_t)out) & 15) ||
+      (((uintptr_t)residual) & 15))
+    return MUSE_ERR_ALIGN;
+  c1x1::Params q;
+  q.gn_partial = nullptr; q.gn_groups = 0; q.gn_cpg = 0;
+  if (gn_partial) {
+    const int cpg = gn_groups > 0 ? Cout / gn_groups : 0;
+    if (gn_groups <= 0 || (Cout % gn_groups) || (cpg & 3) || cpg > 32 || (cpg & (cpg - 1)) || ((H * W) & 127)) return MUSE_ERR_UNSUPPORTED;
+    q.gn_partial = gn_partial; q.gn_groups = gn_groups; q.gn_cpg = cpg;
+  }
+  q.x = in; q.w_hi = w_hi; q.w_lo = w_lo; q.bias = bias; q.residual = residual; q.out = out;
+  q.M = batch * H * W; q.N = Cout; q.K = Cin; q.HW = H * W;
+  const int ntm = (q.M + 127) / 128, ntn = (q.N + 127) / 128;
+  q.nper = ntm >= 1024 ? ntn : 1;
+  const int nsplit = (ntn + q.nper - 1) / q.nper;
+  set_max_dynamic_lds((const void*)conv1x1_split_kernel, c1x1::LDS);
+  hipLaunchKernelGGL(conv1x1_split_kernel, dim3(ntm * nsplit), dim3(256), c1x1::LDS, (hipStream_t)stream, q);
+  return (int)hipGetLastError();
+}
diff --git a/open-muse_amd/csrc/gemm_core.h b/open-muse_amd/csrc/gemm_core.h
--- a/open-muse_amd/csrc/gemm_core.h
+++ b/open-muse_amd/csrc/gemm_core.h
@@ -221,6 +221,27 @@
   }
 };
 
+template <int AL, int BL, int AROWS, int BROWS>
+__device__ __forceinline__ void tile_body_f32(const unsigned char* cA, const unsigned char* cB, int wr, int wc, int lane, f32x4 (&acc)[4][4]) {
+#pragma unroll
+  for (int ks = 0; ks < TileCfg<float>::BK / 16; ++ks) {
+    f32x4 af[4], bf[4];
+#pragma unroll
+    for (int i = 0; i < 4; ++i) {
+      af[i] = frag_f32<AL, AROWS>(cA, wr + i * 16, ks, lane);
+      bf[i] = frag_f32<BL, BROWS>(cB, wc + i * 16, ks, lane);
+    }
+#pragma unroll
+    for (int s = 0; s < 4; ++s)
+#pragma unroll
+      for (int i = 0; i < 4; ++i)
+#pragma unroll
+        for (int j = 0; j < 4; ++j)
+          acc[i][j] = __builtin_amdgcn_mfma_f32_16x16x4f32(bf[j][s], af[i][s], acc[i][j], 0, 0, 0);
+  }
+}
+__device__ __forceinline__ float epilogue_affine(float alpha, float acc, float add) { return alpha * acc + add; }
+
 template <typename T, typename TC, int AL, int BL, int BM, int NSTAGE, typename ALoader, typename BLoader>
 __global__ __launch_bounds__(BM * 2, 2) void gemm_kernel(GemmParams p) {
   using Cfg = TileCfg<T>;
@@ -281,22 +302,7 @@
             acc[i][j] = __builtin_amdgcn_mfma_f32_16x16x32_bf16(bf[j], af[i], acc[i][j], 0, 0, 0);
       }
     } else {
-#pragma unroll
-      for (int ks = 0; ks < Cfg::BK / 16; ++ks) {
-        f32x4 af[4], bf[4];
-#pragma unroll
-        for (int i = 0; i < 4; ++i) {
-          af[i] = frag_f32<AL, BM>(cA, wr + i * 16, ks, lane);
-          bf[i] = frag_f32<BL, 128>(cB, wc + i * 16, ks, lane);
-        }
-#pragma unroll
-        for (int s = 0; s < 4; ++s)
-#pragma unroll
-          for (int i = 0; i < 4; ++i)
-#pragma unroll
-            for (int j = 0; j < 4; ++j)
-              acc[i][j] = __builtin_amdgcn_mfma_f32_16x16x4f32(bf[j][s], af[i][s], acc[i][j], 0, 0, 0);
-      }
+      tile_body_f32<AL, BL, BM, 128>(cA, cB, wr, wc, lane, acc);
     }
   };
 
@@ -389,7 +395,7 @@
               for (int r = 0; r < 4; ++r) {
                 float add = rv;
                 if (p.bias && (n0 + nl + r) < p.N) add += p.bias[n0 + nl + r];
-                float x = p.alpha * acc[i][j][r] + add;
+                float x = epilogue_affine(p.alpha, acc[i][j][r], add);
                 if (p.act == 1) x = gelu_erf(x);
                 v[r] = x;
               }
@@ -458,7 +464,7 @@
       for (int r = 0; r < 4; ++r) {
         float add = rv;
         if (p.bias && (n + r) < p.N) add += p.bias[n + r];
-        float x = p.alpha * acc[i][j][r] + add;
+        float x = epilogue_affine(p.alpha, acc[i][j][r], add);
         if (p.act == 1) x = gelu_erf(x);
         v[r] = x;
       }
diff --git a/open-muse_amd/csrc/vqgan.hip b/open-muse_amd/csrc/vqgan.hip
--- a/open-muse_amd/csrc/vqgan.hip
+++ b/open-muse_amd/csrc/vqgan.hip
@@ -749,18 +749,166 @@
   return (int)hipGetLastError();
 }
 
+__device__ __forceinline__ float row_sumsq_wave(const float* __restrict__ xr, int cols, int lane) {
+  double s = 0.0;
+  for (int c = lane; c < cols; c += 64) { const double v = (double)xr[c]; s += v * v; }
+  return (float)wave_sum_d(s);
+}
 __global__ __launch_bounds__(256) void row_sumsq_kernel(const float* __restrict__ x, float* __restrict__ out, long rows, int cols, long ld) {
   const int lane = threadIdx.x & 63;
   const long row = (long)blockIdx.x * 4 + (threadIdx.x >> 6);
   if (row >= rows) return;
-  double s = 0.0;
-  for (int c = lane; c < cols; c += 64) { const double v = (double)x[row * ld + c]; s += v * v; }
-  s = wave_sum_d(s);
-  if (lane == 0) out[row] = (float)s;
+  const float s = row_sumsq_wave(x + row * ld, cols, lane);
+  if (lane == 0) out[row] = s;
 }
 extern "C" int muse_row_sumsq(const float* x, float* out, int64_t rows, int32_t cols, int64_t ld, void* stream) {
   if (rows <= 0) return 0;
   hipLaunchKernelGGL(row_sumsq_kernel, dim3((unsigned)((rows + 3) / 4)), dim3(256), 0, (hipStream_t)stream, x, out, (long)rows, cols, (long)ld);
+  return (int)hipGetLastError();
+}
+
+namespace vqn {
+constexpr int BM = 64, BN = 256, NT = 256;
+constexpr int TA = BM * TileCfg<float>::KC_STRIDE, TB = BN * TileCfg<float>::KC_STRIDE;
+constexpr int LDS = TA + TB + BM * 4;
+struct Params {
+  const float* z; const float* cb; const float* zn; const float* en; int64_t* idx;
+  long N, ldz, ldc;
+  int Kc, D;
+};
+__device__ __forceinline__ void take(float& best, int& bi, float ov, int oi) {
+  if (ov < best || (ov == best && oi < bi)) { best = ov; bi = oi; }
+}
+}
+__global__ __launch_bounds__(vqn::NT) void vq_nearest_kernel(vqn::Params q) {
+  using namespace vqn;
+  extern __shared__ __attribute__((aligned(16))) unsigned char smem[];
+  unsigned char* tA = smem;
+  unsigned char* tB = smem + TA;
+  float* s_zn = (float*)(smem + TA + TB);
+  const int lane = threadIdx.x & 63, wave = threadIdx.x >> 6;
+  const long m0 = (long)blockIdx.x * BM;
+  const int rows = (int)((q.N - m0) < (long)BM ? (q.N - m0) : (long)BM);
+  const float* zp = q.z + m0 * q.ldz;
+
+  for (int r = wave; r < BM; r += NT / 64) {
+    float v = 0.f;
+    if (r < rows) v = q.zn ? q.zn[m0 + r] : row_sumsq_wave(zp + (long)r * q.ldz, q.D, lane);
+    if (lane == 0) s_zn[r] = v;
+  }
+
+  using ALoader = PlainLoader<float, 0, BM, NT>;
+  using BLoader = PlainLoader<float, 0, BN, NT>;
+  const GemmParams unused{};
+  ALoader la; la.init(zp, q.ldz, rows, q.D, 0, unused);
+  BLoader lb; lb.init(q.cb, q.ldc, q.Kc, q.D, 0, unused);
+  const int nk = q.D / TileCfg<float>::BK, ntile = (q.Kc + BN - 1) / BN;
+  const unsigned tile_bytes = (unsigned)((long)BN * q.ldc * 4);
+
+  u32x4 ra[ALoader::NCH], rb[BLoader::NCH];
+  auto fetch = [&](int t, int kt) {
+#pragma unroll
+    for (int i = 0; i < ALoader::NCH; ++i) ra[i] = la.load(i, kt * TileCfg<float>::BK);
+#pragma unroll
+    for (int i = 0; i < BLoader::NCH; ++i) {
+      const int code = t * BN + (int)(threadIdx.x + NT * i) / BLoader::CPR;
+      rb[i] = buf_load16(lb.rs, code < q.Kc ? lb.voff[i] + (unsigned)t * tile_bytes : lb.oob, (unsigned)(kt * TileCfg<float>::BK) * 4u);
+    }
+  };
+  auto stage = [&]() {
+#pragma unroll
+    for (int i = 0; i < ALoader::NCH; ++i) *(u32x4*)(tA + ALoader::lds_off(i)) = ra[i];
+#pragma unroll
+    for (int i = 0; i < BLoader::NCH; ++i) *(u32x4*)(tB + BLoader::lds_off(i)) = rb[i];
+  };
+
+  const int wc = wave * 64;
+  f32x4 acc[4][4];
+  float best[4]; int bi[4];
+#pragma unroll
+  for (int i = 0; i < 4; ++i) {
+    best[i] = INFINITY; bi[i] = 0x7fffffff;
+#pragma unroll
+    for (int j = 0; j < 4; ++j) acc[i][j] = f32x4{0.f, 0.f, 0.f, 0.f};
+  }
+
+  fetch(0, 0);
+  stage();
+  __syncthreads();
+  float rv[4];
+#pragma unroll
+  for (int i = 0; i < 4; ++i) rv[i] = s_zn[i * 16 + (lane & 15)];
+
+  for (int t = 0; t < ntile; ++t) {
+    for (int kt = 0; kt < nk; ++kt) {
+      const bool last_k = (kt + 1) == nk, more = !last_k || (t + 1) < ntile;
+      if (more) fetch(last_k ? t + 1 : t, last_k ? 0 : kt + 1);
+      tile_body_f32<0, 0, BM, BN>(tA, tB, 0, wc, lane, acc);
+      if (last_k) {
+#pragma unroll
+        for (int j = 0; j < 4; ++j) {
+          const int n = t * BN + wc + j * 16 + 4 * (lane >> 4);
+#pragma unroll
+          for (int r = 0; r < 4; ++r) {
+            if ((n + r) < q.Kc) {
+              const float en = q.en[n + r];
+#pragma unroll
+              for (int i = 0; i < 4; ++i) {
+                float add = rv[i];
+                add += en;
+                const float x = epilogue_affine(-2.0f, acc[i][j][r], add);
+                if (x < best[i]) { best[i] = x; bi[i] = n + r; }
+              }
+            }
+          }
+#pragma unroll
+          for (int i = 0; i < 4; ++i) acc[i][j] = f32x4{0.f, 0.f, 0.f, 0.f};
+        }
+      }
+      __syncthreads();
+      if (more) {
+        stage();
+        __syncthreads();
+      }
+    }
+  }
+
+#pragma unroll
+  for (int i = 0; i < 4; ++i)
+#pragma unroll
+    for (int o = 16; o < 64; o <<= 1) take(best[i], bi[i], __shfl_xor(best[i], o, 64), __shfl_xor(bi[i], o, 64));
+  float* red_v = (float*)smem;
+  int* red_i = (int*)(smem + NT / 64 * BM * 4);
+  if (lane < 16) {
+#pragma unroll
+    for (int i = 0; i < 4; ++i) { red_v[wave * BM + i * 16 + lane] = best[i]; red_i[wave * BM + i * 16 + lane] = bi[i]; }
+  }
+  __syncthreads();
+  if ((int)threadIdx.x < rows) {
+    float b = red_v[threadIdx.x]; int k = red_i[threadIdx.x];
+#pragma unroll
+    for (int w = 1; w < NT / 64; ++w) take(b, k, red_v[w * BM + threadIdx.x], red_i[w * BM + threadIdx.x]);
+    q.idx[m0 + threadIdx.x] = (int64_t)k;
+  }
+}
+extern "C" int muse_vq_nearest_ok(int64_t rows, int32_t ncodes, int32_t dim, int64_t ldz, int64_t ldc) {
+  if (rows < 0 || ncodes < 1 || dim < 64 || (dim & 63)) return 0;
+  if (ldz < dim || ldc < dim || (ldz & 3) || (ldc & 3)) return 0;
+  if ((rows + vqn::BM - 1) / vqn::BM >= (1LL << 31) || ncodes > (1 << 30)) return 0;
+  if (((int64_t)ncodes + vqn::BN) * ldc * 4 >= (1LL << 32) || (int64_t)vqn::BM * ldz * 4 >= (1LL << 32)) return 0;
+  return 1;
+}
+extern "C" int muse_vq_nearest(const float* z, const float* codebook, const float* zn, const float* en, int64_t* idx, int64_t rows,
+                               int32_t ncodes, int32_t dim, int64_t ldz, int64_t ldc, void* stream) {
+  if (!z || !codebook || !en || !idx) return MUSE_ERR_BAD_ARG;
+  if (!muse_vq_nearest_ok(rows, ncodes, dim, ldz, ldc)) return MUSE_ERR_UNSUPPORTED;
+  if ((((uintptr_t)z) & 15) || (((uintptr_t)codebook) & 15)) return MUSE_ERR_ALIGN;
+  if (rows == 0) return 0;
+  vqn::Params q;
+  q.z = z; q.cb = codebook; q.zn = zn; q.en = en; q.idx = idx;
+  q.N = rows; q.ldz = ldz; q.ldc = ldc; q.Kc = ncodes; q.D = dim;
+  set_max_dynamic_lds((const void*)vq_nearest_kernel, vqn::LDS);
+  hipLaunchKernelGGL(vq_nearest_kernel, dim3((unsigned)((rows + vqn::BM - 1) / vqn::BM)), dim3(vqn::NT), vqn::LDS, (hipStream_t)stream, q);
   return (int)hipGetLastError();
 }
 
diff --git a/open-muse_amd/muse/_hip.py b/open-muse_amd/muse/_hip.py
--- a/open-muse_amd/muse/_hip.py
+++ b/open-muse_amd/muse/_hip.py
@@ -141,6 +141,9 @@
                          c_int, c_int, c_void_p],
     "muse_conv2d_nhwc_split": [c_void_p, c_void_p, c_void_p, c_void_p, c_void_p, c_void_p, c_void_p, c_int, c_int, c_int, c_int,
                                c_int, c_int, c_int, c_int, c_void_p],
+    "muse_conv1x1_nhwc_split_ok": [c_int, c_int, c_int, c_int, c_int],
+    "muse_conv1x1_nhwc_split": [c_void_p, c_void_p, c_void_p, c_void_p, c_void_p, c_void_p, c_void_p, c_int, c_int, c_int, c_int,
+                                c_int, c_int, c_void_p],
     "muse_conv2d_nhwc_split2": [c_void_p, c_void_p, c_void_p, c_void_p, c_void_p, c_void_p, c_void_p, c_void_p, c_int, c_int, c_int,
                                 c_int, c_int, c_int, c_int, c_void_p],
     "muse_conv_in_direct": [c_void_p, c_void_p, c_void_p, c_void_p, c_void_p, c_int, c_int, c_int, c_int, c_int, c_int, c_int, c_void_p],
@@ -160,6 +163,8 @@
     "muse_nhwc_to_nchw": [c_void_p, c_int, c_void_p, c_int, c_int, c_int, c_int, c_void_p],
     "muse_argmin_rows": [c_void_p, c_void_p, c_i64, c_int, c_i64, c_void_p],
     "muse_row_sumsq": [c_void_p, c_void_p, c_i64, c_int, c_i64, c_void_p],
+    "muse_vq_nearest_ok": [c_i64, c_int, c_int, c_i64, c_i64],
+    "muse_vq_nearest": [c_void_p, c_void_p, c_void_p, c_void_p, c_void_p, c_i64, c_int, c_int, c_i64, c_i64, c_void_p],
     "muse_gather_rows": [c_void_p, c_void_p, c_void_p, c_int, c_i64, c_int, c_void_p],
     "muse_norm_res_fwd": [c_void_p, c_void_p, c_void_p, c_void_p, c_void_p, c_i64, c_int, c_float, c_int, c_void_p],
     "muse_adaln_fwd": [c_void_p, c_void_p, c_void_p, c_int, c_i64, c_int, c_void_p],
diff --git a/open-muse_amd/muse/modeling_maskgit_vqgan.py b/open-muse_amd/muse/modeling_maskgit_vqgan.py
--- a/open-muse_amd/muse/modeling_maskgit_vqgan.py
+++ b/open-muse_amd/muse/modeling_maskgit_vqgan.py
@@ -112,7 +112,16 @@
         self.dma_conv = True
         self.direct_conv_out = os.environ.get("MUSE_CONV_OUT_DIRECT", "1") != "0"
         self.upsample_split = os.environ.get("MUSE_UPSAMPLE_SPLIT", "1") != "0"
+        self.vq_fused = os.environ.get("MUSE_VQ_FUSED", "1") != "0"
+        self.conv1x1 = os.environ.get("MUSE_CONV1X1", "1") != "0"
         self._packed = {}
+
+    def _drop_packed(self):
+        self._packed = {}
+        ops.drop_codebook_sumsq()
+
+    def _nearest(self, z):
+        return ops.vq_nearest(z, self._codebook(), fused=self.vq_fused, cache_key=self.quantize.embedding.weight)
 
     def _check(self, t):
         if not t.is_cuda:
@@ -122,17 +131,18 @@
         if dtype not in (torch.float32, torch.bfloat16, "bf16x3"):
             raise ValueError('compute dtype must be torch.float32, torch.bfloat16 or "bf16x3"')
         self.compute_dtype = dtype
+        ops.drop_codebook_sumsq()
         return self
 
     def _act_dtype(self):
         return torch.bfloat16 if self.compute_dtype == torch.bfloat16 else torch.float32
 
     def _apply(self, fn, recurse=True):
-        self._packed = {}
+        self._drop_packed()
         return super()._apply(fn, recurse)
 
     def load_state_dict(self, state_dict, strict: bool = True, assign: bool = False):
-        self._packed = {}
+        self._drop_packed()
         return super().load_state_dict(state_dict, strict=strict, assign=assign)
 
     def _cpad(self, c, cd):
@@ -201,6 +211,11 @@
                     and cp == x.shape[-1] and ops.conv_split2_ok(B, H, W, cp, cout, k) and ops.conv_slab_ok(H, W, cp)):
                 hi, lo = ops.split_f32(x)
                 return ops.conv2d_nhwc_split2(hi, lo, wp[0], wp[1], B, H, W, cp, cout, bias=bias, residual=residual,
+                                              gn_groups=32 if (gn_next and self.fuse_gn_stats) else 0)
+            if (self.conv1x1 and k == 1 and not upsample and x.dtype == torch.float32 and x.is_contiguous() and cp == x.shape[-1]
+                    and (residual is None or (residual.dtype == torch.float32 and residual.is_contiguous()))
+                    and ops.conv1x1_split_ok(B, H, W, cp, cout)):
+                return ops.conv1x1_nhwc_split(x, wp[0], wp[1], B, H, W, cp, cout, bias=bias, residual=residual,
                                               gn_groups=32 if (gn_next and self.fuse_gn_stats) else 0)
             return ops.conv2d_nhwc_split(x, wp[0], wp[1], B, H, W, cp, cout, k, bias=bias, residual=residual, upsample=upsample,
                                          gn_groups=32 if (gn_next and self.fuse_gn_stats) else 0)
@@ -351,7 +366,7 @@
     def encode(self, pixel_values, return_loss=False):
         z, (B, H, W) = self._encode_nhwc(pixel_values)
         cb = self._codebook()
-        idx = ops.vq_nearest(z, cb)
+        idx = self._nearest(z)
         zq_rows = ops.gather_rows(cb, idx, torch.float32)
         zq = ops.nhwc_to_nchw(zq_rows.view(B, H, W, -1), zq_rows.shape[1])
         out = (zq, idx.view(B, H * W))
@@ -380,7 +395,7 @@
     @torch.no_grad()
     def get_code(self, pixel_values):
         z, (B, H, W) = self._encode_nhwc(pixel_values)
-        return ops.vq_nearest(z, self._codebook()).view(B, H * W)
+        return self._nearest(z).view(B, H * W)
 
     @torch.no_grad()
     def get_soft_code(self, pixel_values, temp=1.0, stochastic=False):
@@ -388,7 +403,7 @@
         cb = self._codebook()
         soft = ops.vq_neg_distances_scaled(z, cb, 1.0 / float(temp))
         ops.softmax_(soft, soft.shape[0], soft.shape[1], soft.shape[1])
-        code = torch.multinomial(soft, 1) if stochastic else ops.vq_nearest(z, cb)
+        code = torch.multinomial(soft, 1) if stochastic else self._nearest(z)
         return soft.view(B, H * W, -1), code.view(B, H * W)
 
     def forward(self, pixel_values, return_loss=False):
diff --git a/open-muse_amd/muse/modeling_taming_vqgan.py b/open-muse_amd/muse/modeling_taming_vqgan.py
--- a/open-muse_amd/muse/modeling_taming_vqgan.py
+++ b/open-muse_amd/muse/modeling_taming_vqgan.py
@@ -232,7 +232,7 @@
     def encode(self, pixel_values, return_loss=False):
         z, (B, H, W) = self._encode_nhwc(pixel_values)
         cb = self._codebook()
-        idx = ops.vq_nearest(z, cb)
+        idx = self._nearest(z)
         zq_rows = ops.gather_rows(cb, idx, torch.float32)
         zq = ops.nhwc_to_nchw(zq_rows.view(B, H, W, -1), zq_rows.shape[1])
         out = (zq, idx.view(B, H * W))
@@ -260,7 +260,7 @@
     @torch.no_grad()
     def get_code(self, pixel_values):
         z, (B, H, W) = self._encode_nhwc(pixel_values)
-        return ops.vq_nearest(z, self._codebook()).view(B, H * W)
+        return self._nearest(z).view(B, H * W)
 
     @torch.no_grad()
     def get_soft_code(self, pixel_values, temp=1.0, stochastic=False):
@@ -268,7 +268,7 @@
         cb = self._codebook()
         dist = torch.cdist(z, cb).pow(2)
         soft = F.softmax(-dist / temp, dim=-1)
-        code = torch.multinomial(soft, 1) if stochastic else ops.vq_nearest(z, cb)
+        code = torch.multinomial(soft, 1) if stochastic else self._nearest(z)
         return soft.view(B, H * W, -1), code.view(B, H * W)
 
     def forward(self, pixel_values, return_loss=False):
diff --git a/open-muse_amd/muse/ops.py b/open-muse_amd/muse/ops.py
--- a/open-muse_amd/muse/ops.py
+++ b/open-muse_amd/muse/ops.py
@@ -1596,6 +1596,28 @@
     return out
 
 
+def conv1x1_split_ok(B, H, W, Cin, Cout):
+    return bool(lib().muse_conv1x1_nhwc_split_ok(B, H, W, Cin, Cout))
+
+
+def conv1x1_nhwc_split(x, w_hi, w_lo, B, H, W, Cin, Cout, bias=None, residual=None, gn_groups=0):
+    require_gpu(x, w_hi, w_lo)
+    out = torch.empty((B, H, W, Cout), dtype=torch.float32, device=x.device)
+    part, nchunk = None, 0
+    cpg = Cout // gn_groups if gn_groups else 0
+    if gn_groups and Cout % gn_groups == 0 and cpg in (4, 8, 16, 32) and (H * W) % 128 == 0:
+        nchunk = (H * W) // 128
+        part = torch.empty(B * nchunk * gn_groups * 2, dtype=torch.float64, device=out.device)
+    e0 = _prof_begin()
+    check(lib().muse_conv1x1_nhwc_split(x.data_ptr(), w_hi.data_ptr(), w_lo.data_ptr(), ptr(bias), ptr(residual), out.data_ptr(),
+                                        ptr(part), gn_groups if part is not None else 0, B, H, W, Cin, Cout, stream()),
+          "muse_conv1x1_nhwc_split")
+    _prof_end(e0, "conv_bf16x3", 2.0 * B * H * W * Cout * Cin)
+    if part is not None:
+        out._gn_stats = (part, nchunk)
+    return out
+
+
 def conv2d_nhwc_split2(x_hi, x_lo, w_hi, w_lo, B, H, W, Cin, Cout, bias=None, residual=None, gn_groups=0):
     require_gpu(x_hi, x_lo, w_hi, w_lo)
     out = torch.empty((B, H, W, Cout), dtype=torch.float32, device=x_hi.device)
@@ -1835,10 +1857,47 @@
     return out
 
 
-def vq_nearest(z_flat, codebook, en=None, return_dist=False):
+VQ_FUSED = os.environ.get("MUSE_VQ_FUSED", "1") != "0"
+
+_CODEBOOK_SUMSQ = {}
+
+
+def codebook_sumsq(codebook, key=None):
+    require_gpu(codebook)
+    k = codebook if key is None else key
+    sig = (k._version, codebook.data_ptr(), tuple(codebook.shape), codebook.stride())
+    hit = _CODEBOOK_SUMSQ.get(id(k))
+    if hit is not None and hit[0]() is k and hit[1] == sig:
+        return hit[2]
+    Kc, D = codebook.shape
+    en = torch.empty(Kc, dtype=torch.float32, device=codebook.device)
+    check(lib().muse_row_sumsq(codebook.data_ptr(), en.data_ptr(), Kc, D, codebook.stride(0), stream()), "muse_row_sumsq")
+    kid = id(k)
+    _CODEBOOK_SUMSQ[kid] = (weakref.ref(k, lambda _r, kid=kid: _CODEBOOK_SUMSQ.pop(kid, None)), sig, en)
+    return en
+
+
+def drop_codebook_sumsq():
+    _CODEBOOK_SUMSQ.clear()
+
+
+def vq_nearest(z_flat, codebook, en=None, return_dist=False, fused=None, cache_key=None):
     require_gpu(z_flat, codebook)
     N, D = z_flat.shape
     Kc = codebook.shape[0]
+    if fused is None:
+        fused = VQ_FUSED
+    if (fused and not return_dist and z_flat.dtype == torch.float32 and codebook.dtype == torch.float32 and z_flat.stride(1) == 1
+            and codebook.stride(1) == 1 and z_flat.data_ptr() % 16 == 0 and codebook.data_ptr() % 16 == 0
+            and lib().muse_vq_nearest_ok(N, Kc, D, z_flat.stride(0), codebook.stride(0))):
+        if en is None:
+            en = codebook_sumsq(codebook, cache_key)
+        idx = torch.empty(N, dtype=torch.int64, device=z_flat.device)
+        e0 = _prof_begin()
+        check(lib().muse_vq_nearest(z_flat.data_ptr(), codebook.data_ptr(), None, en.data_ptr(), idx.data_ptr(), N, Kc, D,
+                                    z_flat.stride(0), codebook.stride(0), stream()), "muse_vq_nearest")
+        _prof_end(e0, "gemm_f32_NN", 2.0 * N * Kc * D)
+        return idx
     zn = torch.empty(N, dtype=torch.float32, device=z_flat.device)
     check(lib().muse_row_sumsq(z_flat.data_ptr(), zn.data_ptr(), N, D, z_flat.stride(0), stream()), "muse_row_sumsq")
     if en is None:
```
